# deepalcoholic/mlcomp

Measured on AMD Instinct MI355X. Metric: images/sec (whole node) ResNet-50 DAG train task, higher is better.
Workload: dtype bf16; 1 GPU; model=resnet50, global_batch=512, per_gpu_batch=512, image_size=224, parallelism=dp1, impl=native, optimizer=SGD momentum 0.9, wd 5e-5, fp32 master weights

## Files before the change

csrc/kernels/batchnorm.hip:

```cpp
#include "common.h"

namespace {

constexpr int NT = 256;

constexpr int FL = 8;
__global__ void __launch_bounds__(NT)
bn_finalize_kernel(const float* __restrict__ sum, const float* __restrict__ sumsq, int ncopy,
                   const float* __restrict__ gamma, const float* __restrict__ beta,
                   float* __restrict__ save_mean, float* __restrict__ save_invstd,
                   float* __restrict__ scale, float* __restrict__ shift,
                   float* __restrict__ run_mean, float* __restrict__ run_var,
                   long rows, int C, float eps, float momentum) {
  const int c = blockIdx.x * (NT / FL) + (threadIdx.x / FL), q = threadIdx.x % FL;
  float s1 = 0.f, s2 = 0.f;
  if (c < C) {
#pragma unroll 4
    for (int k = q; k < ncopy; k += FL) { s1 += sum[(long)k * C + c]; s2 += sumsq[(long)k * C + c]; }
  }
#pragma unroll
  for (int o = 1; o < FL; o <<= 1) { s1 += __shfl_xor(s1, o, 64); s2 += __shfl_xor(s2, o, 64); }
  if (c >= C || q != 0) return;
  const float inv_count = 1.f / (float)rows;
  const float mean = s1 * inv_count;
  const float var = fmaxf(s2 * inv_count - mean * mean, 0.f);
  const float inv = rsqrtf(var + eps);
  save_mean[c] = mean;
  save_invstd[c] = inv;
  const float g = gamma[c] * inv;
  scale[c] = g;
  shift[c] = beta[c] - mean * g;
  if (run_mean) {
    const float unbiased = rows > 1 ? var * (float)rows / (float)(rows - 1) : var;
    run_mean[c] = (1.f - momentum) * run_mean[c] + momentum * mean;
    run_var[c] = (1.f - momentum) * run_var[c] + momentum * unbiased;
  }
}

template <int U>
__global__ void __launch_bounds__(NT)
bn_fwd_apply_kernel(const bf16* __restrict__ y, const bf16* __restrict__ res, bf16* __restrict__ z,
                    const float* __restrict__ scale_, const float* __restrict__ shift_,
                    const float* __restrict__ rscale_, const float* __restrict__ rshift_,
                    long rows, int C, int relu) {
  const int G = C >> 3;
  const long gtid = (long)blockIdx.x * NT + threadIdx.x;
  const long stride = (long)gridDim.x * NT;
  const int cg = (int)(gtid % G);
  const int c0 = cg * 8;
  float scale[8], shift[8], rscale[8], rshift[8];
#pragma unroll
  for (int j = 0; j < 8; ++j) {
    scale[j] = scale_[c0 + j]; shift[j] = shift_[c0 + j];
    rscale[j] = rscale_ ? rscale_[c0 + j] : 1.f; rshift[j] = rscale_ ? rshift_[c0 + j] : 0.f;
  }
  const long total = rows * G;
  const long last = total - G + cg;
  for (long i0 = gtid; i0 < total; i0 += stride * U) {
    uint4 yv[U], rv[U];
#pragma unroll
    for (int u = 0; u < U; ++u) {
      const long i = min(i0 + u * stride, last);
      yv[u] = *reinterpret_cast<const uint4*>(y + i * 8);
      if (res) rv[u] = *reinterpret_cast<const uint4*>(res + i * 8);
    }
#pragma unroll
    for (int u = 0; u < U; ++u) {
      const long i = i0 + u * stride;
      float f[8];
      unpack8(yv[u], f);
#pragma unroll
      for (int j = 0; j < 8; ++j) f[j] = f[j] * scale[j] + shift[j];
      if (res) {
        float r[8];
        unpack8(rv[u], r);
#pragma unroll
        for (int j = 0; j < 8; ++j) f[j] += r[j] * rscale[j] + rshift[j];
      }
      if (relu) {
#pragma unroll
        for (int j = 0; j < 8; ++j) f[j] = fmaxf(f[j], 0.f);
      }
      if (i < total) *reinterpret_cast<uint4*>(z + i * 8) = pack8(f);
    }
  }
}

constexpr int NSTAT = 32;

__global__ void __launch_bounds__(NT)
bn_bwd_reduce_kernel(const bf16* __restrict__ dz, const bf16* __restrict__ z, const bf16* __restrict__ y,
                     const float* __restrict__ mean, float* __restrict__ sums, long rows, int C, int ncopy) {
  __shared__ float red[2][NT][9];
  const int G = C >> 3;
  const long gtid = (long)blockIdx.x * NT + threadIdx.x;
  const long stride = (long)gridDim.x * NT;
  const int cg = (int)(gtid % G);
  const int c0 = cg * 8;
  float mu[8], s1[8], s2[8];
#pragma unroll
  for (int j = 0; j < 8; ++j) { mu[j] = mean[c0 + j]; s1[j] = 0.f; s2[j] = 0.f; }
  const long total = rows * G;
  constexpr int U = 4;
  for (long i0 = gtid; i0 < total; i0 += stride * U) {
    uint4 dv[U], yv[U], zv[U];
#pragma unroll
    for (int u = 0; u < U; ++u) {
      const long i = i0 + u * stride;
      const long off = (i < total ? i : i0) * 8;
      dv[u] = ldg16(dz + off);
      yv[u] = ldg16(y + off);
      zv[u] = z ? ldg16(z + off) : make_uint4(0u, 0u, 0u, 0u);
    }
#pragma unroll
    for (int u = 0; u < U; ++u) {
      if (i0 + u * stride >= total) break;
      float d[8], yy[8];
      unpack8(dv[u], d);
      unpack8(yv[u], yy);
      if (z) {
        float zz[8];
        unpack8(zv[u], zz);
#pragma unroll
        for (int j = 0; j < 8; ++j) d[j] = zz[j] > 0.f ? d[j] : 0.f;
      }
#pragma unroll
      for (int j = 0; j < 8; ++j) { s1[j] += d[j]; s2[j] += d[j] * (yy[j] - mu[j]); }
    }
  }
  const int t = threadIdx.x;
#pragma unroll
  for (int j = 0; j < 8; ++j) { red[0][t][j] = s1[j]; red[1][t][j] = s2[j]; }
  __syncthreads();
  const int lanes = NT < G ? NT : G;
  const int base_cg = (int)(((long)blockIdx.x * NT) % G);
  float* dst = sums + (size_t)(blockIdx.x % ncopy) * 2 * C;
  if (t < lanes) {
    float a[8], b[8];
#pragma unroll
    for (int j = 0; j < 8; ++j) { a[j] = 0.f; b[j] = 0.f; }
    for (int u = t; u < NT; u += G) {
#pragma unroll
      for (int j = 0; j < 8; ++j) { a[j] += red[0][u][j]; b[j] += red[1][u][j]; }
    }
    const int cgt = (base_cg + t) % G;
#pragma unroll
    for (int j = 0; j < 8; ++j) {
      atomicAdd(dst + cgt * 8 + j, a[j]);
      atomicAdd(dst + C + cgt * 8 + j, b[j]);
    }
  }
}

__global__ void __launch_bounds__(NT)
bn_bwd_finalize_kernel(const float* __restrict__ sums, const float* __restrict__ invstd,
                       const float* __restrict__ gamma, float* __restrict__ coef,
                       float* __restrict__ dgamma, float* __restrict__ dbeta, long rows, int C, int ncopy) {
  const int c = blockIdx.x * (NT / FL) + (threadIdx.x / FL), q = threadIdx.x % FL;
  float S1 = 0.f, S2 = 0.f;
  if (c < C) {
#pragma unroll 4
    for (int k = q; k < ncopy; k += FL) {
      S1 += sums[(size_t)k * 2 * C + c];
      S2 += sums[(size_t)k * 2 * C + C + c];
    }
  }
#pragma unroll
  for (int o = 1; o < FL; o <<= 1) { S1 += __shfl_xor(S1, o, 64); S2 += __shfl_xor(S2, o, 64); }
  if (c >= C || q != 0) return;
  const float invM = 1.f / (float)rows;
  const float is = invstd[c];
  const float k1 = gamma[c] * is;
  coef[c] = k1;
  coef[C + c] = -k1 * S1 * invM;
  coef[2 * C + c] = -k1 * is * is * S2 * invM;
  if (dgamma) { dgamma[c] = S2 * is; dbeta[c] = S1; }
}

template <int U>
__global__ void __launch_bounds__(NT)
bn_bwd_apply_kernel(const bf16* __restrict__ dz, const bf16* __restrict__ z, const bf16* __restrict__ y,
                    const float* __restrict__ mean, const float* __restrict__ coef,
                    bf16* __restrict__ dy, bf16* __restrict__ dres, long rows, int C) {
  const int G = C >> 3;
  const long gtid = (long)blockIdx.x * NT + threadIdx.x;
  const long stride = (long)gridDim.x * NT;
  const int cg = (int)(gtid % G);
  const int c0 = cg * 8;
  float mu[8], k1[8], k2[8], k3[8];
#pragma unroll
  for (int j = 0; j < 8; ++j) {
    mu[j] = mean[c0 + j];
    k1[j] = coef[c0 + j];
    k2[j] = coef[C + c0 + j];
    k3[j] = coef[2 * C + c0 + j];
  }
  const long total = rows * G;
  const long last = total - G + cg;
  for (long i0 = gtid; i0 < total; i0 += stride * U) {
    uint4 dv[U], yv[U], zv[U];
#pragma unroll
    for (int u = 0; u < U; ++u) {
      const long i = min(i0 + u * stride, last);
      dv[u] = *reinterpret_cast<const uint4*>(dz + i * 8);
      yv[u] = *reinterpret_cast<const uint4*>(y + i * 8);
      if (z) zv[u] = *reinterpret_cast<const uint4*>(z + i * 8);
    }
#pragma unroll
    for (int u = 0; u < U; ++u) {
      const long i = i0 + u * stride;
      float d[8], yy[8], o[8];
      unpack8(dv[u], d);
      unpack8(yv[u], yy);
      if (z) {
        float zz[8];
        unpack8(zv[u], zz);
#pragma unroll
        for (int j = 0; j < 8; ++j) d[j] = zz[j] > 0.f ? d[j] : 0.f;
      }
      if (i < total) {
        if (dres) *reinterpret_cast<uint4*>(dres + i * 8) = pack8(d);
#pragma unroll
        for (int j = 0; j < 8; ++j) o[j] = k1[j] * d[j] + k2[j] + k3[j] * (yy[j] - mu[j]);
        *reinterpret_cast<uint4*>(dy + i * 8) = pack8(o);
      }
    }
  }
}

constexpr int FG = 32;

__device__ __forceinline__ void fused_geom(int G, int& gb, int& nslices) {
  gb = slice_groups(G, FG);
  nslices = G / gb;
}

__device__ __forceinline__ void fused_reduce(const float* __restrict__ a, const float* __restrict__ b, long stride,
                                             int ncopy, int c0, int nch, int t, float (&red)[2][NT]) {
  const int P = NT / nch, p = t / nch, cl = t % nch;
  float x = 0.f, y = 0.f;
  if (p < P) {
#pragma unroll 16
    for (int k = p; k < ncopy; k += P) { x += a[k * stride + c0 + cl]; y += b[k * stride + c0 + cl]; }
  }
  red[0][t] = x;
  red[1][t] = y;
  __syncthreads();
  if (t < nch) {
    for (int q = 1; q < P; ++q) { x += red[0][q * nch + t]; y += red[1][q * nch + t]; }
  }
  __syncthreads();
  if (t < nch) { red[0][t] = x; red[1][t] = y; }
  __syncthreads();
}

template <int U>
__global__ void __launch_bounds__(NT)
bn_fwd_fused_kernel(const bf16* __restrict__ y, const bf16* __restrict__ res, bf16* __restrict__ z,
                    const float* __restrict__ sum, const float* __restrict__ sumsq, int ncopy,
                    const float* __restrict__ gamma, const float* __restrict__ beta,
                    float* __restrict__ save_mean, float* __restrict__ save_invstd,
                    float* __restrict__ scale_out, float* __restrict__ shift_out,
                    float* __restrict__ run_mean, float* __restrict__ run_var,
                    const float* __restrict__ rscale_, const float* __restrict__ rshift_,
                    long rows, int C, float eps, float momentum, int relu) {
  __shared__ float lsc[FG * 8], lsh[FG * 8], red[2][NT];
  const int G = C >> 3;
  int gb, nslices;
  fused_geom(G, gb, nslices);
  const int slice = blockIdx.x % nslices, part = blockIdx.x / nslices, nparts = gridDim.x / nslices;
  const int t = threadIdx.x, nch = gb * 8, c0 = slice * nch;
  fused_reduce(sum, sumsq, (long)C, ncopy, c0, nch, t, red);
  if (t < nch) {
    const int c = c0 + t;
    const float s1 = red[0][t], s2 = red[1][t];
    const float inv_count = 1.f / (float)rows;
    const float mean = s1 * inv_count;
    const float var = fmaxf(s2 * inv_count - mean * mean, 0.f);
    const float inv = rsqrtf(var + eps);
    const float g = gamma[c] * inv, h = beta[c] - mean * g;
    lsc[t] = g;
    lsh[t] = h;
    if (part == 0) {
      save_mean[c] = mean;
      save_invstd[c] = inv;
      scale_out[c] = g;
      shift_out[c] = h;
      if (run_mean) {
        const float unbiased = rows > 1 ? var * (float)rows / (float)(rows - 1) : var;
        run_mean[c] = (1.f - momentum) * run_mean[c] + momentum * mean;
        run_var[c] = (1.f - momentum) * run_var[c] + momentum * unbiased;
      }
    }
  }
  __syncthreads();
  const int rpi = NT / gb;
  if (t >= rpi * gb) return;
  const int g = t % gb, cg = slice * gb + g;
  float sc[8], sh[8], rsc[8], rsh[8];
#pragma unroll
  for (int j = 0; j < 8; ++j) {
    sc[j] = lsc[g * 8 + j];
    sh[j] = lsh[g * 8 + j];
    rsc[j] = rscale_ ? rscale_[cg * 8 + j] : 1.f;
    rsh[j] = rscale_ ? rshift_[cg * 8 + j] : 0.f;
  }
  const long step = (long)nparts * rpi;
  for (long r0 = (long)part * rpi + t / gb; r0 < rows; r0 += step * U) {
    uint4 yv[U], rv[U];
#pragma unroll
    for (int u = 0; u < U; ++u) {
      const long r = min(r0 + u * step, rows - 1);
      yv[u] = ldg16(y + (r * G + cg) * 8);
      rv[u] = res ? ldg16(res + (r * G + cg) * 8) : make_uint4(0u, 0u, 0u, 0u);
    }
#pragma unroll
    for (int u = 0; u < U; ++u) {
      const long r = r0 + u * step;
      if (r >= rows) break;
      float f[8];
      unpack8(yv[u], f);
#pragma unroll
      for (int j = 0; j < 8; ++j) f[j] = f[j] * sc[j] + sh[j];
      if (res) {
        float q[8];
        unpack8(rv[u], q);
#pragma unroll
        for (int j = 0; j < 8; ++j) f[j] += q[j] * rsc[j] + rsh[j];
      }
      if (relu) {
#pragma unroll
        for (int j = 0; j < 8; ++j) f[j] = fmaxf(f[j], 0.f);
      }
      *reinterpret_cast<uint4*>(z + (r * G + cg) * 8) = pack8(f);
    }
  }
}

template <int U>
__global__ void __launch_bounds__(NT)
bn_bwd_fused_kernel(const bf16* __restrict__ dz, const bf16* __restrict__ z, const bf16* __restrict__ y,
                    const float* __restrict__ mean, const float* __restrict__ sums, int ncopy,
                    const float* __restrict__ invstd, const float* __restrict__ gamma,
                    float* __restrict__ dgamma, float* __restrict__ dbeta, bf16* __restrict__ dy,
                    bf16* __restrict__ dres, long rows, int C) {
  __shared__ float lk[3][FG * 8], lmu[FG * 8], red[2][NT];
  const int G = C >> 3;
  int gb, nslices;
  fused_geom(G, gb, nslices);
  const int slice = blockIdx.x % nslices, part = blockIdx.x / nslices, nparts = gridDim.x / nslices;
  const int t = threadIdx.x, nch = gb * 8, c0 = slice * nch;
  fused_reduce(sums, sums + C, 2L * C, ncopy, c0, nch, t, red);
  if (t < nch) {
    const int c = c0 + t;
    const float S1 = red[0][t], S2 = red[1][t];
    const float invM = 1.f / (float)rows;
    const float is = invstd[c];
    const float k1 = gamma[c] * is;
    lk[0][t] = k1;
    lk[1][t] = -k1 * S1 * invM;
    lk[2][t] = -k1 * is * is * S2 * invM;
    lmu[t] = mean[c];
    if (part == 0 && dgamma) { dgamma[c] = S2 * is; dbeta[c] = S1; }
  }
  __syncthreads();
  const int rpi = NT / gb;
  if (t >= rpi * gb) return;
  const int g = t % gb, cg = slice * gb + g;
  float k1[8], k2[8], k3[8], mu[8];
#pragma unroll
  for (int j = 0; j < 8; ++j) {
    k1[j] = lk[0][g * 8 + j];
    k2[j] = lk[1][g * 8 + j];
    k3[j] = lk[2][g * 8 + j];
    mu[j] = lmu[g * 8 + j];
  }
  const long step = (long)nparts * rpi;
  for (long r0 = (long)part * rpi + t / gb; r0 < rows; r0 += step * U) {
    uint4 dv[U], yv[U], zv[U];
#pragma unroll
    for (int u = 0; u < U; ++u) {
      const long r = min(r0 + u * step, rows - 1);
      const long i = r * G + cg;
      dv[u] = ldg16(dz + i * 8);
      yv[u] = ldg16(y + i * 8);
      zv[u] = z ? ldg16(z + i * 8) : make_uint4(0u, 0u, 0u, 0u);
    }
#pragma unroll
    for (int u = 0; u < U; ++u) {
      const long r = r0 + u * step;
      if (r >= rows) break;
      const long i = r * G + cg;
      float d[8], yy[8], o[8];
      unpack8(dv[u], d);
      unpack8(yv[u], yy);
      if (z) {
        float zz[8];
        unpack8(zv[u], zz);
#pragma unroll
        for (int j = 0; j < 8; ++j) d[j] = zz[j] > 0.f ? d[j] : 0.f;
      }
      if (dres) *reinterpret_cast<uint4*>(dres + i * 8) = pack8(d);
#pragma unroll
      for (int j = 0; j < 8; ++j) o[j] = k1[j] * d[j] + k2[j] + k3[j] * (yy[j] - mu[j]);
      *reinterpret_cast<uint4*>(dy + i * 8) = pack8(o);
    }
  }
}

int g_unroll = 1;
int g_max_blocks = 512;
int g_fused = 1;

long grid_mult(int G) {
  if (G > NT) return G / NT;
  int a = G, b = NT;
  while (b) { const int r = a % b; a = b; b = r; }
  return G / a;
}

int grid_for(long rows, int C) {
  const int G = C >> 3;
  long total = rows * G;
  long blocks = (total + NT * 4 - 1) / (NT * 4);
  if (blocks > g_max_blocks) blocks = g_max_blocks;
  if (blocks < 1) blocks = 1;
  const long m = grid_mult(G);
  blocks = ((blocks + m - 1) / m) * m;
  return (int)blocks;
}

int fused_grid(long rows, int C) {
  const int G = C >> 3;
  const int gb = slice_groups(G, FG), nslices = G / gb;
  const int rpi = NT / gb;
  long parts = (rows + (long)rpi * 4 - 1) / ((long)rpi * 4);
  long cap = g_max_blocks / nslices;
  if (cap < 1) cap = 1;
  if (parts > cap) parts = cap;
  if (parts < 1) parts = 1;
  return (int)(parts * nslices);
}

bool fused_ok(int C, int ncopy) {
  const int G = C >> 3;
  if (g_fused != 1 || C % 8 || ncopy < 1 || ncopy > 64) return false;
  return G >= 1;
}

bool shape_ok(int C) {
  const int G = C >> 3;
  if (C % 8) return false;
  return G <= NT || G % NT == 0;
}

}

int g_mlc_ncopy = NSTAT;
int g_mlc_det = 0;

MLC_EXPORT int mlc_set_deterministic(int det, int ncopy) {
  g_mlc_det = det ? 1 : 0;
  g_mlc_ncopy = ncopy >= NSTAT ? ncopy : NSTAT;
  return 0;
}
MLC_EXPORT int mlc_get_stat_copies() { return g_mlc_ncopy; }
MLC_EXPORT int mlc_get_deterministic() { return g_mlc_det; }

MLC_EXPORT int mlc_bn_finalize(const float* sum, const float* sumsq, int ncopy, const float* gamma,
                               const float* beta, float* save_mean, float* save_invstd, float* scale,
                               float* shift, float* run_mean, float* run_var, long rows, int C,
                               float eps, float momentum, hipStream_t st) {
  hipLaunchKernelGGL(bn_finalize_kernel, dim3((C + NT / FL - 1) / (NT / FL)), dim3(NT), 0, st, sum, sumsq, ncopy,
                     gamma, beta, save_mean, save_invstd, scale, shift, run_mean, run_var, rows, C, eps,
                     momentum);
  return hipGetLastError();
}

MLC_EXPORT int mlc_bn_fwd_apply2(const bf16* y, const bf16* res, bf16* z, const float* scale,
                                 const float* shift, const float* rscale, const float* rshift, long rows,
                                 int C, int relu, hipStream_t st) {
  if (!shape_ok(C) || (rscale && !rshift)) return -1;
  const dim3 grid(grid_for(rows, C));
  if (g_unroll >= 4)
    hipLaunchKernelGGL(bn_fwd_apply_kernel<4>, grid, dim3(NT), 0, st, y, res, z, scale, shift, rscale, rshift,
                       rows, C, relu);
  else if (g_unroll == 2)
    hipLaunchKernelGGL(bn_fwd_apply_kernel<2>, grid, dim3(NT), 0, st, y, res, z, scale, shift, rscale, rshift,
                       rows, C, relu);
  else
    hipLaunchKernelGGL(bn_fwd_apply_kernel<1>, grid, dim3(NT), 0, st, y, res, z, scale, shift, rscale, rshift,
                       rows, C, relu);
  return hipGetLastError();
}

MLC_EXPORT int mlc_bn_fwd_apply(const bf16* y, const bf16* res, bf16* z, const float* scale,
                                const float* shift, long rows, int C, int relu, hipStream_t st) {
  return mlc_bn_fwd_apply2(y, res, z, scale, shift, nullptr, nullptr, rows, C, relu, st);
}

MLC_EXPORT int mlc_bn_bwd_reduce(const bf16* dz, const bf16* z, const bf16* y, const float* mean,
                                 float* sums, long rows, int C, hipStream_t st) {
  if (!shape_ok(C)) return -1;
  int blocks = grid_for(rows, C);
  const int G = C >> 3;
  if (G >= 64) {
    int cap = 65536 / G;
    if (cap < 256) cap = 256;
    const long m = grid_mult(G);
    cap = (int)(((cap + m - 1) / m) * m);
    if (blocks > cap) blocks = cap;
  }
  if (g_mlc_det && blocks > g_mlc_ncopy) return -2;
  hipLaunchKernelGGL(bn_bwd_reduce_kernel, dim3(blocks), dim3(NT), 0, st, dz, z, y,
                     mean, sums, rows, C, g_mlc_ncopy);
  return hipGetLastError();
}

MLC_EXPORT int mlc_bn_bwd_finalize(const float* sums, const float* invstd, const float* gamma,
                                   float* coef, float* dgamma, float* dbeta, long rows, int C,
                                   hipStream_t st) {
  hipLaunchKernelGGL(bn_bwd_finalize_kernel, dim3((C + NT / FL - 1) / (NT / FL)), dim3(NT), 0, st, sums, invstd,
                     gamma, coef, dgamma, dbeta, rows, C, g_mlc_ncopy);
  return hipGetLastError();
}

MLC_EXPORT int mlc_bn_fwd_fused(const bf16* y, const bf16* res, bf16* z, const float* sum, const float* sumsq,
                                int ncopy, const float* gamma, const float* beta, float* save_mean,
                                float* save_invstd, float* scale, float* shift, float* run_mean, float* run_var,
                                const float* rscale, const float* rshift, long rows, int C, float eps,
                                float momentum, int relu, hipStream_t st) {
  if (!fused_ok(C, ncopy) || (rscale && !rshift) || rows < 1) return -1;
#define MLC_BNF(U) hipLaunchKernelGGL(bn_fwd_fused_kernel<U>, dim3(fused_grid(rows, C)), dim3(NT), 0, st, y, res, z, \
                                      sum, sumsq, ncopy, gamma, beta, save_mean, save_invstd, scale, shift, run_mean, \
                                      run_var, rscale, rshift, rows, C, eps, momentum, relu)
  if (g_unroll >= 4) MLC_BNF(4); else if (g_unroll == 2) MLC_BNF(2); else MLC_BNF(1);
#undef MLC_BNF
  return hipGetLastError();
}

MLC_EXPORT int mlc_bn_bwd_fused(const bf16* dz, const bf16* z, const bf16* y, const float* mean, const float* sums,
                                int ncopy, const float* invstd, const float* gamma, float* dgamma, float* dbeta,
                                bf16* dy, bf16* dres, long rows, int C, hipStream_t st) {
  if (!fused_ok(C, ncopy) || rows < 1) return -1;
#define MLC_BNB(U) hipLaunchKernelGGL(bn_bwd_fused_kernel<U>, dim3(fused_grid(rows, C)), dim3(NT), 0, st, dz, z, y, \
                                      mean, sums, ncopy, invstd, gamma, dgamma, dbeta, dy, dres, rows, C)
  if (g_unroll >= 4) MLC_BNB(4); else if (g_unroll == 2) MLC_BNB(2); else MLC_BNB(1);
#undef MLC_BNB
  return hipGetLastError();
}

MLC_EXPORT int mlc_bn_bwd_apply(const bf16* dz, const bf16* z, const bf16* y, const float* mean,
                                const float* coef, bf16* dy, bf16* dres, long rows, int C,
                                hipStream_t st) {
  if (!shape_ok(C)) return -1;
  const dim3 grid(grid_for(rows, C));
  if (g_unroll >= 4)
    hipLaunchKernelGGL(bn_bwd_apply_kernel<4>, grid, dim3(NT), 0, st, dz, z, y, mean, coef, dy, dres, rows, C);
  else if (g_unroll == 2)
    hipLaunchKernelGGL(bn_bwd_apply_kernel<2>, grid, dim3(NT), 0, st, dz, z, y, mean, coef, dy, dres, rows, C);
  else
    hipLaunchKernelGGL(bn_bwd_apply_kernel<1>, grid, dim3(NT), 0, st, dz, z, y, mean, coef, dy, dres, rows, C);
  return hipGetLastError();
}

MLC_EXPORT int mlc_bn_get_set(int key, int value) {
  int* k = key == 0 ? &g_unroll : key == 1 ? &g_max_blocks : key == 2 ? &g_fused : nullptr;
  if (!k) return -1;
  const int old = *k;
  if (value > 0) *k = value;
  return old;
}
```

csrc/kernels/common.h:

```cpp
#pragma once
#include <hip/hip_runtime.h>
#include <stdint.h>

typedef __bf16 bf16;
typedef __bf16 bf16x8 __attribute__((ext_vector_type(8)));
typedef __bf16 bf16x4 __attribute__((ext_vector_type(4)));
typedef __bf16 bf16x2 __attribute__((ext_vector_type(2)));
typedef short s16x4 __attribute__((ext_vector_type(4)));
typedef float f32x16 __attribute__((ext_vector_type(16)));
typedef float f32x4 __attribute__((ext_vector_type(4)));

#define LDS_PTR(T) __attribute__((address_space(3))) T*

#define MLC_EXPORT extern "C" __attribute__((visibility("default")))

extern int g_mlc_ncopy;
extern int g_mlc_det;
extern "C" int mlc_bn_stats(const bf16* x, float* sum, float* sumsq, long rows, int C, hipStream_t st);

static __device__ __forceinline__ float bf2f(bf16 v) { return (float)v; }
static __device__ __forceinline__ bf16 f2bf(float v) { return (bf16)v; }

static __host__ __device__ __forceinline__ int slice_groups(int G, int cap) {
  int d = G < cap ? G : cap;
  while (d > 1 && G % d) --d;
  return d;
}

static __device__ __forceinline__ void unpack8(const uint4& u, float* f) {
  const uint32_t w[4] = {u.x, u.y, u.z, u.w};
#pragma unroll
  for (int i = 0; i < 4; ++i) {
    f[2 * i] = __uint_as_float(w[i] << 16);
    f[2 * i + 1] = __uint_as_float(w[i] & 0xffff0000u);
  }
}

static __device__ __forceinline__ uint32_t pack2_bf16(float a, float b) {
  const bf16x2 r = {(bf16)a, (bf16)b};
  return __builtin_bit_cast(uint32_t, r);
}
static __device__ __forceinline__ uint32_t f2bf_bits(float f) {
  return (uint32_t)__builtin_bit_cast(unsigned short, (bf16)f);
}

static __device__ __forceinline__ uint4 pack8(const float* f) {
  uint4 r;
  r.x = pack2_bf16(f[0], f[1]);
  r.y = pack2_bf16(f[2], f[3]);
  r.z = pack2_bf16(f[4], f[5]);
  r.w = pack2_bf16(f[6], f[7]);
  return r;
}

static __device__ __forceinline__ uint4 ldg16(const void* p) {
  typedef unsigned u32x4 __attribute__((ext_vector_type(4)));
  const u32x4 v = *reinterpret_cast<const u32x4*>(p);
  return make_uint4(v.x, v.y, v.z, v.w);
}
static __device__ __forceinline__ void ldg8f(const float* p, float* f) {
  typedef float f32x4v __attribute__((ext_vector_type(4)));
  const f32x4v a = *reinterpret_cast<const f32x4v*>(p), b = *reinterpret_cast<const f32x4v*>(p + 4);
  f[0] = a.x; f[1] = a.y; f[2] = a.z; f[3] = a.w; f[4] = b.x; f[5] = b.y; f[6] = b.z; f[7] = b.w;
}

static __device__ __forceinline__ float wave_sum(float v) {
#pragma unroll
  for (int o = 32; o > 0; o >>= 1) v += __shfl_xor(v, o, 64);
  return v;
}

static __device__ __forceinline__ int xcd_remap(int orig, int nwg) {
  const int q = nwg >> 3, r = nwg & 7;
  const int xcd = orig & 7, loc = orig >> 3;
  return (xcd < r ? xcd * (q + 1) : r * (q + 1) + (xcd - r) * q) + loc;
}

static __global__ void __launch_bounds__(256) mlc_zero_f32_kernel(float* __restrict__ p, long n) {
  for (long i = (long)blockIdx.x * 256 + threadIdx.x; i < n; i += (long)gridDim.x * 256) p[i] = 0.f;
}
static inline void mlc_zero_f32(float* p, long n, hipStream_t st) {
  if (n <= 0) return;
  long blocks = (n + 255) / 256;
  if (blocks > 4096) blocks = 4096;
  hipLaunchKernelGGL(mlc_zero_f32_kernel, dim3(blocks), dim3(256), 0, st, p, n);
}
```

csrc/kernels/igemm.hip:

```cpp
#include "gfx950.h"
#include "convgeom.h"
#include <stdlib.h>
#include <map>
#include <mutex>
#include <vector>
#include <algorithm>
#include <cstdio>

namespace igemm {

constexpr int BK = 64, NTHR = 256;


template <int R>
__device__ __forceinline__ int mc_off(int k, int c) {
  if (R == 64) return k * 128 + ((c ^ (((k >> 1) & 1) << 2)) << 4);
  return k * (R * 2) + ((c ^ ((k & 3) << 2)) << 4);
}

template <class L, int R>
__device__ __forceinline__ void store_stage(char* lds, int tid, const uint4 (&v)[R / 32]) {
#pragma unroll
  for (int i = 0; i < R / 32; ++i) *reinterpret_cast<uint4*>(lds + L::lds_off(i, tid)) = v[i];
}
// ... 366 lines not shown
#pragma unroll
      for (int c = 0; c < NC; ++c) {
        const bool ok = (unsigned)(hb + st.rd[c]) < (unsigned)g.H && (unsigned)(wb + st.sd[c]) < (unsigned)g.W;
        v[2 * c + j] = bload(rsr, ok ? rel + st.coff[c] : OOB);
      }
    }
  }
};

struct BnIn { const float* sc; const float* sh; };
template <class L, class = void> struct HasXform { static constexpr bool value = false; };
template <class L> struct HasXform<L, decltype((void)L::XF)> { static constexpr bool value = L::XF; };
template <class L, class = void> struct HasDma { static constexpr bool value = false; };
template <class L> struct HasDma<L, decltype((void)L::DMA)> {
  static constexpr bool value = L::DMA && !HasXform<L>::value && !HasSum<L>::value;
};

__device__ __forceinline__ uint4 bn_relu8(uint4 v, const float* a, const float* b, bool ok) {
  float f[8];
  unpack8(v, f);
#pragma unroll
  for (int e = 0; e < 8; ++e) f[e] = fmaxf(f[e] * a[e] + b[e], 0.f);
  const uint4 r = pack8(f);
  return ok ? r : make_uint4(0u, 0u, 0u, 0u);
}

template <int R>
struct MatKCBn : MatKC<R> {
  static constexpr bool XF = true;
  BnIn bn;
  __device__ void xform(const typename MatKC<R>::St& st, int kt, int tid, uint4 (&v)[R / 32]) const {
    const int c0 = kt * BK + (tid & 7) * 8;
    const bool kv = c0 < this->K;
    float a[8], b[8];
    ldg8f(bn.sc + (kv ? c0 : 0), a);
    ldg8f(bn.sh + (kv ? c0 : 0), b);
#pragma unroll
    for (int i = 0; i < R / 32; ++i) v[i] = bn_relu8(v[i], a, b, kv && st.off[i] != OOB);
  }
};

template <int R>
struct ConvFwdABn : ConvFwdA<R> {
  static constexpr bool XF = true;
  BnIn bn;
  __device__ void xform(const typename ConvFwdA<R>::St& st, int kt, int tid, uint4 (&v)[R / 32]) const {
    const ConvGeom& g = this->g;
    const int k0 = kt * BK, k = k0 + (tid & 7) * 8;
    unsigned rs_, cc, rr, ss;
    if (g.C % BK == 0) {
      g.fC.divmod((unsigned)k0, rs_, cc);
      cc += (unsigned)(k - k0);
    } else {
      g.fC.divmod((unsigned)k, rs_, cc);
    }
    g.fKW.divmod(rs_, rr, ss);
    const bool kv = k < this->K;
    const unsigned P = kv ? tap_pat((int)rr, (int)ss) : NO_TAP;
    float a[8], b[8];
    ldg8f(bn.sc + (kv ? cc : 0), a);
    ldg8f(bn.sh + (kv ? cc : 0), b);
#pragma unroll
    for (int i = 0; i < R / 32; ++i) v[i] = bn_relu8(v[i], a, b, (st.msk[i] & P) == P);
  }
};

template <int R>
struct MatMCBn : MatMC<R> {
  static constexpr bool XF = true;
  BnIn bn;
  __device__ void xform(const typename MatMC<R>::St& st, int kt, int tid, uint4 (&v)[R / 32]) const {
    const int c0 = st.n0 + (tid % (R / 8)) * 8;
    const bool cv = c0 < this->cols;
    float a[8], b[8];
    ldg8f(bn.sc + (cv ? c0 : 0), a);
    ldg8f(bn.sh + (cv ? c0 : 0), b);
    const int left = this->K - kt * BK;
#pragma unroll
    for (int i = 0; i < R / 32; ++i) v[i] = bn_relu8(v[i], a, b, cv && MatMC<R>::kr(i, tid) < left);
  }
};

template <int R>
struct ConvWgradBBn : ConvWgradB<R> {
  static constexpr bool XF = true;
  BnIn bn;
  __device__ void xform(const typename ConvWgradB<R>::St& st, int kt, int tid, uint4 (&v)[R / 32]) const {
    constexpr int NC = ConvWgradB<R>::NC;
    const ConvGeom& g = this->g;
    const int p0 = kt * BK;
    unsigned t, w0, n0, h0;
    g.fWo.divmod((unsigned)p0, t, w0);
    g.fHo.divmod(t, n0, h0);
    int hb[2], wb[2];
#pragma unroll
    for (int j = 0; j < 2; ++j) {
      const int kr = (tid >> 3) + 32 * j;
      unsigned cw, wo, ch, ho;
      g.fWo.divmod(w0 + (unsigned)kr, cw, wo);
      g.fHo.divmod(h0 + cw, ch, ho);
      hb[j] = p0 + kr < this->P ? (int)ho * g.stride - g.pad : -(1 << 29);
      wb[j] = (int)wo * g.stride - g.padw;
    }
#pragma unroll
    for (int c = 0; c < NC; ++c) {
      float a[8], b[8];
      ldg8f(bn.sc + st.ci[c], a);
      ldg8f(bn.sh + st.ci[c], b);
#pragma unroll
      for (int j = 0; j < 2; ++j) {
        const bool ok = (unsigned)(hb[j] + st.rd[c]) < (unsigned)g.H && (unsigned)(wb[j] + st.sd[c]) < (unsigned)g.W;
        v[2 * c + j] = bn_relu8(v[2 * c + j], a, b, ok);
      }
    }
  }
};


struct IdentityRows {
  __device__ __forceinline__ size_t operator()(int m) const { return (size_t)m; }
};
struct ClassRows {
  DgradClass c; int H, W;
  __device__ __forceinline__ size_t operator()(int m) const {
    int n, i, j;
    c.decode(m, n, i, j);
    return ((size_t)n * H + i * c.S + c.ph) * W + j * c.S + c.pw;
  }
};
template <class Rows = IdentityRows>
struct StridedAddRows {
  Rows rows; int Ho, Wo; FastDiv fW, fH, fS;
  __device__ __forceinline__ size_t operator()(int m) const { return rows(m); }
  __device__ __forceinline__ bool addend_pixel(size_t pix, size_t& cpix) const {
    unsigned t, n, h, w, hq, hr, wq, wr;
    fW.divmod((unsigned)pix, t, w);
    fH.divmod(t, n, h);
    fS.divmod(h, hq, hr);
    fS.divmod(w, wq, wr);
    cpix = ((size_t)n * Ho + hq) * Wo + wq;
    return (hr | wr) == 0;
  }
};
template <class R> struct HasStridedAdd { static constexpr bool value = false; };
template <class R> struct HasStridedAdd<StridedAddRows<R>> { static constexpr bool value = true; };

struct BnBwdEpi {
  const bf16* mask = nullptr;
  const bf16* y0 = nullptr; const float* mean0 = nullptr; float* sums0 = nullptr;
  const bf16* y1 = nullptr; const float* mean1 = nullptr; float* sums1 = nullptr;
  const float* msc0 = nullptr; const float* msh0 = nullptr;
  const float* msc1 = nullptr; const float* msh1 = nullptr;
  int ncopy = NSTAT;
};

__device__ __forceinline__ float erf_from_exp(float x, float e) {
  const float t = __builtin_amdgcn_rcpf(1.f + 0.3275911f * fabsf(x));
  const float p = ((((1.061405429f * t - 1.453152027f) * t + 1.421413741f) * t - 0.284496736f) * t + 0.254829592f) * t;
  return copysignf(1.f - p * e, x);
}

__device__ __forceinline__ void dense_act8(float (&a)[8], int act, bf16* pre) {
  const int mode = act & 3;
  if (mode == 3) {
    if (pre) *reinterpret_cast<uint4*>(pre) = pack8(a);
#pragma unroll
    for (int e = 0; e < 8; ++e) a[e] = fmaxf(a[e], 0.f);
    return;
  }
  if (mode == 2) {
    float d[8];
#pragma unroll
    for (int e = 0; e < 8; ++e) {
      const float u = a[e];
      const float ex = __expf(-0.5f * u * u);
      const float cdf = 0.5f * (1.f + erf_from_exp(u * 0.70710678118654752f, ex));
      d[e] = cdf + u * 0.3989422804014327f * ex;
      a[e] = u * cdf;
    }
    if (pre) *reinterpret_cast<uint4*>(pre) = pack8(d);
    return;
  }
  if (pre) *reinterpret_cast<uint4*>(pre) = pack8(a);
  if (mode == 1) {
#pragma unroll
    for (int e = 0; e < 8; ++e)
      a[e] = 0.5f * a[e] * (1.f + erf_from_exp(a[e] * 0.70710678118654752f, __expf(-0.5f * a[e] * a[e])));
  }
}
__device__ __forceinline__ void dense_dact8(float (&a)[8], int act, uint4 zv) {
  float z[8];
  unpack8(zv, z);
  if (act & 4) {
#pragma unroll
    for (int e = 0; e < 8; ++e) a[e] *= z[e];
    return;
  }
  if ((act & 3) == 3) {
#pragma unroll
    for (int e = 0; e < 8; ++e) a[e] = z[e] > 0.f ? a[e] : 0.f;
    return;
  }
#pragma unroll
  for (int e = 0; e < 8; ++e) {
    const float ex = __expf(-0.5f * z[e] * z[e]);
    const float cdf = 0.5f * (1.f + erf_from_exp(z[e] * 0.70710678118654752f, ex));
    a[e] *= cdf + z[e] * 0.3989422804014327f * ex;
  }
}

template <class RowMap = IdentityRows, bool kDense = false>
struct EpiBF16 {
  bf16* out; int ld; float* sum; float* sumsq; RowMap rowmap; const bf16* addend = nullptr;
  BnBwdEpi bn = {};
  const float* bias = nullptr; int act = 0; bf16* preact = nullptr; const bf16* dact = nullptr;
  int ncopy = NSTAT;
  bool raw_sync = false;
  __device__ __forceinline__ void esync() const {
    if (raw_sync) lds_barrier();
    else __syncthreads();
  }
  template <int BM, int BN, int MI, int NI>
  __device__ void apply(f32x16 (&acc)[MI][NI], char* lds, int m0, int n0, int M, int N,
                        int wm, int wn, int lane, int tid) const {
    if (sum) {
      const int slot = (int)((unsigned)((m0 / 64) + wm) % (unsigned)ncopy);
#pragma unroll
      for (int j = 0; j < NI; ++j) {
        float s1 = 0.f, s2 = 0.f;
#pragma unroll
        for (int i = 0; i < MI; ++i)
#pragma unroll
          for (int r = 0; r < 16; ++r) { const float v = acc[i][j][r]; s1 += v; s2 += v * v; }
        s1 += __shfl_xor(s1, 32, 64);
        s2 += __shfl_xor(s2, 32, 64);
        const int n = n0 + wn * 32 * NI + 32 * j + lane;
        if (lane < 32 && n < N) {
          atomicAdd(sum + (size_t)slot * N + n, s1);
          atomicAdd(sumsq + (size_t)slot * N + n, s2);
        }
      }
    }
    constexpr int RS = (BN + 8) * 2;
    esync();
#pragma unroll
    for (int i = 0; i < MI; ++i)
#pragma unroll
      for (int j = 0; j < NI; ++j)
#pragma unroll
        for (int r = 0; r < 16; ++r) {
          const int m = wm * 32 * MI + 32 * i + (r & 3) + 8 * (r >> 2) + 4 * (lane >> 5);
          const int n = wn * 32 * NI + 32 * j + (lane & 31);
          *reinterpret_cast<bf16*>(lds + m * RS + n * 2) = (bf16)acc[i][j][r];
        }
    esync();
    constexpr int CPR = BN / 8;
    constexpr int RPI = NTHR / CPR;
    constexpr bool EXACT = RPI * CPR == NTHR && BM % RPI == 0;
    const bool tok = EXACT || tid < RPI * CPR;
    const int c = tid % CPR;
    const int nc = n0 + c * 8;
    const bool red = !kDense && bn.y0 != nullptr;
    float mu0[8], mu1[8], s1[8], s2[8], t2[8], ma0[8], mb0[8], ma1[8], mb1[8];
    const bool aff = red && !bn.mask && bn.msc0, aff1 = aff && bn.msc1;
    if (red) {
      const int ncl = nc < N ? nc : 0;
#pragma unroll
      for (int e = 0; e < 8; ++e) {
        s1[e] = 0.f; s2[e] = 0.f; t2[e] = 0.f;
        mu1[e] = 0.f; ma0[e] = 0.f; mb0[e] = 0.f; ma1[e] = 0.f; mb1[e] = 0.f;
      }
      ldg8f(bn.mean0 + ncl, mu0);
      if (bn.y1) ldg8f(bn.mean1 + ncl, mu1);
      if (aff) { ldg8f(bn.msc0 + ncl, ma0); ldg8f(bn.msh0 + ncl, mb0); }
      if (aff1) { ldg8f(bn.msc1 + ncl, ma1); ldg8f(bn.msh1 + ncl, mb1); }
    }
    const bool dense = kDense && (bias || act || dact);
    float bz[8];
#pragma unroll
    for (int e = 0; e < 8; ++e) bz[e] = 0.f;
    if (kDense && bias) ldg8f(bias + (nc < N ? nc : 0), bz);
    constexpr int ITERS = (BM + RPI - 1) / RPI;
    if (!addend && !red && !dense) {
#pragma unroll
      for (int it = 0; it < ITERS; ++it) {
        const int row = tid / CPR + RPI * it;
        const int m = m0 + row;
        if ((EXACT || (tok && row < BM)) && m < M && nc < N)
          *reinterpret_cast<uint4*>(out + rowmap(m) * ld + nc) =
              *reinterpret_cast<const uint4*>(lds + row * RS + c * 16);
      }
      return;
    }
    constexpr int UMAX = kDense ? 4 : 8;
    constexpr int U = ITERS < UMAX ? ITERS : UMAX;
    const bool has_add = addend != nullptr, has_mask = red && bn.mask, has_y1 = red && bn.y1;
    constexpr bool kSAdd = HasStridedAdd<RowMap>::value;
#pragma unroll 1
    for (int it0 = 0; it0 < ITERS; it0 += U) {
      constexpr int UB = kDense ? 1 : U;
      constexpr int UD = kDense ? U : 1;
      uint4 vv[U], aa[U], zz[UB], p0[UB], p1[UB], du[UD];
      size_t off[U];
      bool ok[U], hit[U];
#pragma unroll
      for (int u = 0; u < U; ++u) {
        int row = tid / CPR + RPI * (it0 + u);
        const bool rin = EXACT || (tok && row < BM);
        if (!rin) row = 0;
        const int m = m0 + row;
        ok[u] = rin && m < M && nc < N;
        const size_t pix = ok[u] ? rowmap(m) : 0;
        off[u] = ok[u] ? pix * ld + nc : 0;
        vv[u] = *reinterpret_cast<const uint4*>(lds + row * RS + c * 16);
        const uint4 zero = make_uint4(0u, 0u, 0u, 0u);
        if constexpr (kSAdd) {
          size_t cpix = 0;
          hit[u] = has_add && ok[u] && rowmap.addend_pixel(pix, cpix);
          aa[u] = hit[u] ? ldg16(addend + cpix * ld + nc) : zero;
        } else {
          hit[u] = has_add;
          aa[u] = has_add ? ldg16(addend + off[u]) : zero;
        }
        if constexpr (!kDense) {
          zz[u] = has_mask ? ldg16(bn.mask + off[u]) : zero;
          p0[u] = red ? ldg16(bn.y0 + off[u]) : zero;
          p1[u] = has_y1 ? ldg16(bn.y1 + off[u]) : zero;
        }
        if constexpr (kDense) du[u] = dact ? ldg16(dact + off[u]) : zero;
      }
#pragma unroll
      for (int u = 0; u < U; ++u) {
        if (!ok[u]) continue;
        uint4 v = vv[u];
        if (has_add || red || dense) {
          float a[8];
          unpack8(v, a);
          if constexpr (kDense) {
          if (bias) {
#pragma unroll
            for (int e = 0; e < 8; ++e) a[e] += bz[e];
          }
          dense_act8(a, act, preact ? preact + off[u] : nullptr);
          if (dact) dense_dact8(a, act, du[u]);
          }
          if (hit[u]) {
            float b[8];
            unpack8(aa[u], b);
#pragma unroll
            for (int e = 0; e < 8; ++e) a[e] += b[e];
          }
          if constexpr (!kDense) {
            if (has_mask) {
              float z[8];
              unpack8(zz[u], z);
#pragma unroll
              for (int e = 0; e < 8; ++e) a[e] = z[e] > 0.f ? a[e] : 0.f;
            } else if (aff) {
              float y[8], q[8];
              unpack8(p0[u], y);
#pragma unroll
              for (int e = 0; e < 8; ++e) q[e] = y[e] * ma0[e] + mb0[e];
              if (aff1) {
                unpack8(p1[u], y);
#pragma unroll
                for (int e = 0; e < 8; ++e) q[e] += y[e] * ma1[e] + mb1[e];
              }
#pragma unroll
              for (int e = 0; e < 8; ++e) a[e] = q[e] > 0.f ? a[e] : 0.f;
            }
          }
          v = pack8(a);
          if constexpr (!kDense) if (red) {
            unpack8(v, a);
            float y[8];
            unpack8(p0[u], y);
#pragma unroll
            for (int e = 0; e < 8; ++e) { s1[e] += a[e]; s2[e] += a[e] * (y[e] - mu0[e]); }
            if (has_y1) {
              unpack8(p1[u], y);
#pragma unroll
              for (int e = 0; e < 8; ++e) t2[e] += a[e] * (y[e] - mu1[e]);
            }
          }
        }
        *reinterpret_cast<uint4*>(out + off[u]) = v;
      }
    }
    if (red) {
      float* rb = reinterpret_cast<float*>(lds);
      esync();
#pragma unroll
      for (int e = 0; e < 8; ++e) {
        rb[tid * 24 + e] = s1[e];
        rb[tid * 24 + 8 + e] = s2[e];
        rb[tid * 24 + 16 + e] = t2[e];
      }
      esync();
      if (tid < BN) {
        const int col = tid, cc = col >> 3, e = col & 7, n = n0 + col;
        float a = 0.f, b = 0.f, d = 0.f;
        for (int r = 0; r < RPI; ++r) {
          const float* q = rb + (cc + CPR * r) * 24;
          a += q[e]; b += q[8 + e]; d += q[16 + e];
        }
        if (n < N) {
          const int slot = (int)((unsigned)(m0 / BM) % (unsigned)bn.ncopy);
          float* d0 = bn.sums0 + (size_t)slot * 2 * N;
          atomicAdd(d0 + n, a);
          atomicAdd(d0 + N + n, b);
          if (bn.y1) {
            float* d1 = bn.sums1 + (size_t)slot * 2 * N;
            atomicAdd(d1 + n, a);
            atomicAdd(d1 + N + n, d);
          }
        }
      }
    }
  }
};

struct EpiF32Slab {
  float* ws; int ld; size_t slab;
  template <int BM, int BN, int MI, int NI>
  __device__ void apply(f32x16 (&acc)[MI][NI], char*, int m0, int n0, int M, int N,
                        int wm, int wn, int lane, int) const {
    float* out = ws + (size_t)blockIdx.z * slab;
#pragma unroll
    for (int i = 0; i < MI; ++i)
#pragma unroll
      for (int j = 0; j < NI; ++j) {
        const int n = n0 + wn * 32 * NI + 32 * j + (lane & 31);
        if (n >= N) continue;
#pragma unroll
        for (int r = 0; r < 16; ++r) {
          const int m = m0 + wm * 32 * MI + 32 * i + (r & 3) + 8 * (r >> 2) + 4 * (lane >> 5);
          if (m < M) out[(size_t)m * ld + n] = acc[i][j][r];
        }
      }
  }
};


struct DenseFinish {
  bf16* C; int ldc; const float* bias; int act; bf16* preact; const bf16* addend; const bf16* dact;
  __device__ __forceinline__ void run(const float* ws, size_t slab, int splits, size_t src, int m, int c) const {
    typedef float v4 __attribute__((ext_vector_type(4)));
    const float* base = ws + src;
    v4 lo = {0.f, 0.f, 0.f, 0.f}, hi = {0.f, 0.f, 0.f, 0.f};
    int k = 0;
    for (; k + 2 <= splits; k += 2) {
      const v4 p0 = *reinterpret_cast<const v4*>(base + k * slab);
      const v4 q0 = *reinterpret_cast<const v4*>(base + k * slab + 4);
      const v4 p1 = *reinterpret_cast<const v4*>(base + (k + 1) * slab);
      const v4 q1 = *reinterpret_cast<const v4*>(base + (k + 1) * slab + 4);
      lo += p0 + p1;
      hi += q0 + q1;
    }
    if (k < splits) {
      lo += *reinterpret_cast<const v4*>(base + k * slab);
      hi += *reinterpret_cast<const v4*>(base + k * slab + 4);
    }
    float a[8] = {lo.x, lo.y, lo.z, lo.w, hi.x, hi.y, hi.z, hi.w};
    const size_t o = (size_t)m * ldc + c;
    if (bias) {
      float bz[8];
      ldg8f(bias + c, bz);
#pragma unroll
      for (int e = 0; e < 8; ++e) a[e] += bz[e];
    }
    dense_act8(a, act, preact ? preact + o : nullptr);
    if (dact) dense_dact8(a, act, ldg16(dact + o));
    if (addend) {
      float b[8];
      unpack8(ldg16(addend + o), b);
#pragma unroll
      for (int e = 0; e < 8; ++e) a[e] += b[e];
    }
    *reinterpret_cast<uint4*>(C + o) = pack8(a);
  }
};

struct EpiSlabFused {
  float* ws; int ld; size_t slab; unsigned* cnt;
  int dense;
  float* outf; int accumulate;
  DenseFinish fin;
  template <int BM, int BN, int MI, int NI>
  __device__ void apply(f32x16 (&acc)[MI][NI], char* lds, int m0, int n0, int M, int N,
                        int wm, int wn, int lane, int tid) const {
    float* part = ws + (size_t)blockIdx.z * slab;
#pragma unroll
    for (int i = 0; i < MI; ++i)
#pragma unroll
      for (int j = 0; j < NI; ++j) {
        const int n = n0 + wn * 32 * NI + 32 * j + (lane & 31);
        if (n >= N) continue;
#pragma unroll
        for (int r = 0; r < 16; ++r) {
          const int m = m0 + wm * 32 * MI + 32 * i + (r & 3) + 8 * (r >> 2) + 4 * (lane >> 5);
          if (m < M) part[(size_t)m * ld + n] = acc[i][j][r];
        }
      }
    vmwait<0>();
    __syncthreads();
    int* flag = reinterpret_cast<int*>(lds);
    if (tid == 0) {
      __builtin_amdgcn_fence(__ATOMIC_RELEASE, "agent");
      vmwait<0>();
      const unsigned t = __hip_atomic_fetch_add(cnt + blockIdx.x, 1u, __ATOMIC_RELAXED, __HIP_MEMORY_SCOPE_AGENT);
// ... 636 lines not shown

struct MkMatKC {
  const bf16* p; int ld, rows, K;
  template <int R> MatKC<R> make() const { return MatKC<R>{p, ld, rows, K}; }
};
struct MkMatMC {
  const bf16* p; int ld, K, cols;
  template <int R> MatMC<R> make() const { return MatMC<R>{p, ld, K, cols}; }
};
struct MkMatMCSum {
  const bf16* p; int ld, K, cols; float* colsum;
  template <int R> MatMCSum<R> make() const { return MatMCSum<R>{p, ld, K, cols, colsum}; }
};
struct MkMatKCBn {
  const bf16* p; int ld, rows, K; BnIn bn;
  template <int R> MatKCBn<R> make() const { return MatKCBn<R>{{p, ld, rows, K}, bn}; }
};
struct MkMatMCBn {
  const bf16* p; int ld, K, cols; BnIn bn;
  template <int R> MatMCBn<R> make() const { return MatMCBn<R>{{p, ld, K, cols}, bn}; }
};
struct MkConvFwdA {
  const bf16* x; ConvGeom g; int M, K;
  template <int R> ConvFwdA<R> make() const { return ConvFwdA<R>{x, g, M, K}; }
};
struct MkConvFwdABn {
  const bf16* x; ConvGeom g; int M, K; BnIn bn;
  template <int R> ConvFwdABn<R> make() const { return ConvFwdABn<R>{{x, g, M, K}, bn}; }
};
struct MkConvDgradA {
  const bf16* dy; ConvGeom g; int M, K; DgradClass cl;
  template <int R> ConvDgradA<R> make() const { return ConvDgradA<R>{dy, g, M, K, cl}; }
};
struct MkConvDgradB {
  const bf16* w; ConvGeom g; DgradClass cl;
  template <int R> ConvDgradB<R> make() const { return ConvDgradB<R>{w, g, cl}; }
};
struct MkConvDgradBT {
  const bf16* wt; ConvGeom g; DgradClass cl;
  template <int R> ConvDgradBT<R> make() const { return ConvDgradBT<R>{wt, g, cl}; }
};
struct MkConvWgradB {
  const bf16* x; ConvGeom g; int P, KK;
  template <int R> ConvWgradB<R> make() const { return ConvWgradB<R>{x, g, P, KK}; }
};
struct MkConvWgradBBn {
  const bf16* x; ConvGeom g; int P, KK; BnIn bn;
  template <int R> ConvWgradBBn<R> make() const { return ConvWgradBBn<R>{{x, g, P, KK}, bn}; }
};

template <class EPI, class FA, class FB>
static hipError_t launch_tiles(int tile, int M, int N, int K, int splits, hipStream_t st, const EPI& epi,
                               const FA& fa, const FB& fb) {
  if (tile == 1) return launch<256, 64>(fa.template make<256>(), fb.template make<64>(), epi, M, N, K, splits, st);
  if (tile == 2) return launch<64, 256>(fa.template make<64>(), fb.template make<256>(), epi, M, N, K, splits, st);
  if (tile == 3) return launch<256, 128>(fa.template make<256>(), fb.template make<128>(), epi, M, N, K, splits, st);
  if (tile == 4) return launch<128, 256>(fa.template make<128>(), fb.template make<256>(), epi, M, N, K, splits, st);
  return launch<128, 128>(fa.template make<128>(), fb.template make<128>(), epi, M, N, K, splits, st);
}

template <class EPI, class FA, class FB>
static hipError_t launch_dense_tiles(int dt, int M, int N, int K, int splits, hipStream_t st, const EPI& epi,
                                     const FA& fa, const FB& fb) {
  if (dt == 5) return launch<128, 96>(fa.template make<128>(), fb.template make<96>(), epi, M, N, K, splits, st);
  if (dt == 6) return launch<128, 192>(fa.template make<128>(), fb.template make<192>(), epi, M, N, K, splits, st);
  return launch<128, 288>(fa.template make<128>(), fb.template make<288>(), epi, M, N, K, splits, st);
}

template <class EPI>
static hipError_t dispatch_ab(int ta, int tb, const bf16* A, int lda, const bf16* B, int ldb, int tile, int M, int N,
                              int K, int splits, hipStream_t st, const EPI& epi) {
  const MkMatKC a_kc{A, lda, M, K}, b_kc{B, ldb, N, K};
  const MkMatMC a_mc{A, lda, K, M}, b_mc{B, ldb, K, N};
  if (!ta && tb) return launch_tiles(tile, M, N, K, splits, st, epi, a_kc, b_kc);
  if (!ta && !tb) return launch_tiles(tile, M, N, K, splits, st, epi, a_kc, b_mc);
  if (ta && tb) return launch_tiles(tile, M, N, K, splits, st, epi, a_mc, b_kc);
  return launch_tiles(tile, M, N, K, splits, st, epi, a_mc, b_mc);
}

MLC_EXPORT int mlc_bn_stat_copies() { return NSTAT; }

MLC_EXPORT int mlc_gemm_config(int prefetch) {
  const int old = igemm::g_prefetch;
  if (prefetch == 1 || prefetch == 2) igemm::g_prefetch = prefetch;
  return old;
}

MLC_EXPORT int mlc_gemm_get_set(int key, int value) {
  static int* const knobs[] = {
      &g_prefetch, &g_split_target, &g_split_target_mat, &g_big_tiles, &g_big_min_blocks, &g_single_stage,
      &g_splitk_fused, &g_dense_narrow, &g_gemm_dma, &g_split_target_dense, &g_dense_tile, &g_dense_split,
      &g_dense_bf16_split_target, &g_single_stage_kt, &g_persist, &g_persist_nbuf, &g_persist_kt};
  if (key < 0 || key >= (int)(sizeof(knobs) / sizeof(knobs[0]))) return -1;
  int* k = knobs[key];
  if (key == 14) resolve_persist_defaults();
  if (key == 10 || key == 11) {
    int sp = 1;
    (void)pick_dense_tile(4096, 768, 768, sp);
  }
  const int old = *k;
  if (key == 10) {
    if (value >= -1) *k = value;
    return old;
  }
  if (value >= 0 && (value > 0 || key == 3 || key == 5 || key == 6 || key == 7 || key == 8 || key == 12)) *k = value;
  return old;
}

static int conv_fwd_impl(const bf16* x, const bf16* w, bf16* y, int ldy, float* sum, float* sumsq,
                         int N, int H, int W, int C, int Co, int KH, int KW, int stride,
                         int pad, int dil, int Ho, int Wo, const float* in_sc, const float* in_sh,
                         hipStream_t st) {
  if (C % 8 || Co % 8 || ldy < Co || ldy % 8 || KH > 15 || KW > 16 || ((in_sc == nullptr) != (in_sh == nullptr)))
    return -1;
  const int M = N * Ho * Wo, K = KH * KW * C;
  const int tile = pick_tile(M, Co);
  EpiBF16<> epi{y, ldy, sum, sumsq, IdentityRows{}};
  epi.ncopy = g_mlc_ncopy;
  if (sum && g_mlc_det && (M + 63) / 64 > g_mlc_ncopy) return -2;
  const BnIn bn{in_sc, in_sh};
  const MkMatKC fb{w, K, Co, K};
  if (KH == 1 && KW == 1 && stride == 1 && pad == 0) {
    if (in_sc) return launch_tiles(tile, M, Co, K, 1, st, epi, MkMatKCBn{x, C, M, K, bn}, fb);
    return launch_tiles(tile, M, Co, K, 1, st, epi, MkMatKC{x, C, M, K}, fb);
  }
  const ConvGeom g = mkgeom(N, H, W, C, Co, KH, KW, stride, pad, dil, Ho, Wo);
  if (in_sc) return launch_tiles(tile, M, Co, K, 1, st, epi, MkConvFwdABn{x, g, M, K, bn}, fb);
  return launch_tiles(tile, M, Co, K, 1, st, epi, MkConvFwdA{x, g, M, K}, fb);
}

MLC_EXPORT int mlc_conv_fwd(const bf16* x, const bf16* w, bf16* y, float* sum, float* sumsq,
                            int N, int H, int W, int C, int Co, int KH, int KW, int stride,
                            int pad, int dil, int Ho, int Wo, const float* in_sc, const float* in_sh,
                            hipStream_t st) {
  return conv_fwd_impl(x, w, y, Co, sum, sumsq, N, H, W, C, Co, KH, KW, stride, pad, dil, Ho, Wo, in_sc, in_sh, st);
}

MLC_EXPORT int mlc_conv_fwd_ld(const bf16* x, const bf16* w, bf16* y, int ldy, int N, int H, int W, int C, int Co,
                               int KH, int KW, int stride, int pad, int dil, int Ho, int Wo, hipStream_t st) {
  return conv_fwd_impl(x, w, y, ldy, nullptr, nullptr, N, H, W, C, Co, KH, KW, stride, pad, dil, Ho, Wo, nullptr,
                       nullptr, st);
}

struct DgradAddend {
  const bf16* same = nullptr; const bf16* compact = nullptr; int S = 1;
};

static int dgrad_check(const BnBwdEpi& bn, const DgradAddend& add, int N, int H, int W, int C, int Co, int KH,
                       int KW, int stride, const float* sum, const float* sumsq) {
  if (C % 8 || Co % 8 || KH > 15 || KW > 16 || stride < 1 || ((sum == nullptr) != (sumsq == nullptr))) return -1;
  if (add.S < 1 || (add.compact && add.same)) return -1;
  if (bn.y0 && g_mlc_det && ((long)N * H * W + 63) / 64 > g_mlc_ncopy) return -2;
  if (bn.msc0 && (!bn.msh0 || !bn.y0 || (bn.msc1 && (!bn.msh1 || !bn.y1)))) return -1;
  if (bn.y0 && (!bn.mean0 || !bn.sums0 || (bn.y1 && (!bn.mean1 || !bn.sums1)))) return -1;
  return 0;
}

template <class Rows, class FA, class FB>
static hipError_t launch_dgrad(const Rows& rows, bf16* dx, const DgradAddend& add, const BnBwdEpi& bn, float* sum,
                               float* sumsq, int H, int W, int M, int C, int K, hipStream_t st, const FA& fa,
                               const FB& fb) {
  const int tile = pick_tile(M, C);
  if (add.compact) {
    const StridedAddRows<Rows> srows{rows, (H - 1) / add.S + 1, (W - 1) / add.S + 1, FastDiv(W), FastDiv(H),
                                     FastDiv(add.S)};
    EpiBF16<StridedAddRows<Rows>> epi{dx, C, sum, sumsq, srows, add.compact, bn};
    epi.ncopy = g_mlc_ncopy;
    return launch_tiles(tile, M, C, K, 1, st, epi, fa, fb);
  }
  EpiBF16<Rows> epi{dx, C, sum, sumsq, rows, add.same, bn};
  epi.ncopy = g_mlc_ncopy;
  return launch_tiles(tile, M, C, K, 1, st, epi, fa, fb);
}

template <class MkB>
static int dgrad_classes(const bf16* dy, const bf16* w, bf16* dx, const DgradAddend& add, const BnBwdEpi& bn,
                         const ConvGeom& g, int pad, float* sum, float* sumsq, hipStream_t st) {
  hipError_t err = hipSuccess;
  for (int ph = 0; ph < g.stride && ph < g.H; ++ph)
    for (int pw = 0; pw < g.stride && pw < g.W; ++pw) {
      const DgradClass cl = mkclass(g.stride, ph, pw, g.H, g.W, g.Ho, g.Wo, g.Co, g.KH, g.KW, pad, g.dil);
      if (cl.nr > 15 || cl.ns > 16) return -1;
      const int M = g.N * cl.Hc * cl.Wc, K = cl.nr * cl.ns * cl.ncb * BK;
      if (M <= 0) continue;
      if (sum && g_mlc_det && (M + 63) / 64 > g_mlc_ncopy) return -2;
      const MkConvDgradA fa{dy, g, M, K, cl};
      const MkB fb{w, g, cl};
      if (g.stride == 1)
        err = launch_dgrad(IdentityRows{}, dx, add, bn, sum, sumsq, g.H, g.W, M, g.C, K, st, fa, fb);
      else
        err = launch_dgrad(ClassRows{cl, g.H, g.W}, dx, add, bn, sum, sumsq, g.H, g.W, M, g.C, K, st, fa, fb);
      if (err != hipSuccess) return err;
    }
  return err;
}

static int conv_dgrad_impl(const bf16* dy, const bf16* w, bf16* dx, const DgradAddend& add, int N,
                           int H, int W, int C, int Co, int KH, int KW, int stride, int pad,
                           int dil, int Ho, int Wo, const bf16* bn_mask, const bf16* bn_y0,
                           const float* bn_mean0, float* bn_sums0, const bf16* bn_y1,
                           const float* bn_mean1, float* bn_sums1, const float* bn_msc0,
                           const float* bn_msh0, const float* bn_msc1, const float* bn_msh1,
                           float* sum, float* sumsq, hipStream_t st) {
  const BnBwdEpi bn{bn_mask, bn_y0, bn_mean0, bn_sums0, bn_y1, bn_mean1, bn_sums1,
                    bn_msc0, bn_msh0, bn_msc1, bn_msh1, g_mlc_ncopy};
  if (const int rc = dgrad_check(bn, add, N, H, W, C, Co, KH, KW, stride, sum, sumsq)) return rc;
  const ConvGeom g = mkgeom(N, H, W, C, Co, KH, KW, stride, pad, dil, Ho, Wo);
  if (KH == 1 && KW == 1 && stride == 1 && pad == 0) {
    const DgradClass cl = mkclass(1, 0, 0, H, W, Ho, Wo, Co, 1, 1, 0, dil);
    const int M = N * H * W, K = cl.ncb * BK;
    if (sum && g_mlc_det && (M + 63) / 64 > g_mlc_ncopy) return -2;
    return launch_dgrad(IdentityRows{}, dx, add, bn, sum, sumsq, H, W, M, C, K, st, MkMatKC{dy, Co, M, Co},
                        MkConvDgradB{w, g, cl});
  }
  return dgrad_classes<MkConvDgradB>(dy, w, dx, add, bn, g, pad, sum, sumsq, st);
}

MLC_EXPORT int mlc_conv_dgrad(const bf16* dy, const bf16* w, bf16* dx, const bf16* addend, int N,
                              int H, int W, int C, int Co, int KH, int KW, int stride, int pad,
                              int dil, int Ho, int Wo, const bf16* bn_mask, const bf16* bn_y0,
                              const float* bn_mean0, float* bn_sums0, const bf16* bn_y1,
                              const float* bn_mean1, float* bn_sums1, const float* bn_msc0,
                              const float* bn_msh0, const float* bn_msc1, const float* bn_msh1,
                              hipStream_t st) {
  return conv_dgrad_impl(dy, w, dx, DgradAddend{addend}, N, H, W, C, Co, KH, KW, stride, pad, dil, Ho, Wo, bn_mask,
                         bn_y0, bn_mean0, bn_sums0, bn_y1, bn_mean1, bn_sums1, bn_msc0, bn_msh0, bn_msc1, bn_msh1,
                         nullptr, nullptr, st);
}

MLC_EXPORT int mlc_conv_dgrad_sadd(const bf16* dy, const bf16* w, bf16* dx, const bf16* addend, const bf16* sadd,
                                   int sadd_stride, int N, int H, int W, int C, int Co, int KH, int KW,
                                   int stride, int pad, int dil, int Ho, int Wo, const bf16* bn_mask,
                                   const bf16* bn_y0, const float* bn_mean0, float* bn_sums0, const bf16* bn_y1,
                                   const float* bn_mean1, float* bn_sums1, const float* bn_msc0,
                                   const float* bn_msh0, const float* bn_msc1, const float* bn_msh1,
                                   hipStream_t st) {
  return conv_dgrad_impl(dy, w, dx, DgradAddend{addend, sadd, sadd_stride}, N, H, W, C, Co, KH, KW, stride, pad, dil,
                         Ho, Wo, bn_mask, bn_y0, bn_mean0, bn_sums0, bn_y1, bn_mean1, bn_sums1, bn_msc0, bn_msh0,
                         bn_msc1, bn_msh1, nullptr, nullptr, st);
}

MLC_EXPORT int mlc_conv_tr_fwd(const bf16* x, const bf16* w, bf16* y, float* sum, float* sumsq, int N, int Hi,
                               int Wi, int Cin, int Cout, int KH, int KW, int stride, int pad, int dil, int Ho,
                               int Wo, hipStream_t st) {
  int pad_h, pad_w;
  unpack_pad(pad, pad_h, pad_w);
  if (Hi != (Ho + 2 * pad_h - dil * (KH - 1) - 1) / stride + 1 || Wi != (Wo + 2 * pad_w - dil * (KW - 1) - 1) / stride + 1)
    return -1;
  return conv_dgrad_impl(x, w, y, DgradAddend{}, N, Ho, Wo, Cout, Cin, KH, KW, stride, pad, dil, Hi, Wi, nullptr,
                         nullptr, nullptr, nullptr, nullptr, nullptr, nullptr, nullptr, nullptr, nullptr,
                         nullptr, sum, sumsq, st);
}

static int conv_dgrad_t_impl(const bf16* dy, const bf16* wt, bf16* dx, const DgradAddend& add, int N,
                             int H, int W, int C, int Co, int KH, int KW, int stride, int pad,
                             int dil, int Ho, int Wo, const bf16* bn_mask, const bf16* bn_y0,
                             const float* bn_mean0, float* bn_sums0, const bf16* bn_y1,
                             const float* bn_mean1, float* bn_sums1, const float* bn_msc0,
                             const float* bn_msh0, const float* bn_msc1, const float* bn_msh1,
                             hipStream_t st) {
  const BnBwdEpi bn{bn_mask, bn_y0, bn_mean0, bn_sums0, bn_y1, bn_mean1, bn_sums1,
                    bn_msc0, bn_msh0, bn_msc1, bn_msh1, g_mlc_ncopy};
  if (const int rc = dgrad_check(bn, add, N, H, W, C, Co, KH, KW, stride, nullptr, nullptr)) return rc;
  int pad_h, pad_w;
  unpack_pad(pad, pad_h, pad_w);
  const int ph = dil * (KH - 1) - pad_h, pw = dil * (KW - 1) - pad_w;
  if (stride == 1 && ph >= 0 && pw >= 0) {
    if (Ho != H + 2 * pad_h - dil * (KH - 1) || Wo != W + 2 * pad_w - dil * (KW - 1)) return -1;
    const int M = N * H * W, K = KH * KW * Co;
    const MkMatKC fb{wt, K, C, K};
    if (KH == 1 && KW == 1)
      return launch_dgrad(IdentityRows{}, dx, add, bn, nullptr, nullptr, H, W, M, C, K, st, MkMatKC{dy, Co, M, Co},
                          fb);
    const ConvGeom gf = mkgeom(N, Ho, Wo, Co, C, KH, KW, 1, pack_pad(ph, pw), dil, H, W);
    return launch_dgrad(IdentityRows{}, dx, add, bn, nullptr, nullptr, H, W, M, C, K, st, MkConvFwdA{dy, gf, M, K},
                        fb);
  }
  const ConvGeom g = mkgeom(N, H, W, C, Co, KH, KW, stride, pad, dil, Ho, Wo);
  return dgrad_classes<MkConvDgradBT>(dy, wt, dx, add, bn, g, pad, nullptr, nullptr, st);
}

MLC_EXPORT int mlc_conv_dgrad_t(const bf16* dy, const bf16* wt, bf16* dx, const bf16* addend, int N,
                                int H, int W, int C, int Co, int KH, int KW, int stride, int pad,
                                int dil, int Ho, int Wo, const bf16* bn_mask, const bf16* bn_y0,
                                const float* bn_mean0, float* bn_sums0, const bf16* bn_y1,
                                const float* bn_mean1, float* bn_sums1, const float* bn_msc0,
                                const float* bn_msh0, const float* bn_msc1, const float* bn_msh1,
                                hipStream_t st) {
  return conv_dgrad_t_impl(dy, wt, dx, DgradAddend{addend}, N, H, W, C, Co, KH, KW, stride, pad, dil, Ho, Wo,
                           bn_mask, bn_y0, bn_mean0, bn_sums0, bn_y1, bn_mean1, bn_sums1, bn_msc0, bn_msh0, bn_msc1,
                           bn_msh1, st);
}

MLC_EXPORT int mlc_conv_dgrad_t_sadd(const bf16* dy, const bf16* wt, bf16* dx, const bf16* addend, const bf16* sadd,
                                     int sadd_stride, int N, int H, int W, int C, int Co, int KH, int KW,
                                     int stride, int pad, int dil, int Ho, int Wo, const bf16* bn_mask,
                                     const bf16* bn_y0, const float* bn_mean0, float* bn_sums0, const bf16* bn_y1,
                                     const float* bn_mean1, float* bn_sums1, const float* bn_msc0,
                                     const float* bn_msh0, const float* bn_msc1, const float* bn_msh1,
                                     hipStream_t st) {
  return conv_dgrad_t_impl(dy, wt, dx, DgradAddend{addend, sadd, sadd_stride}, N, H, W, C, Co, KH, KW, stride, pad,
                           dil, Ho, Wo, bn_mask, bn_y0, bn_mean0, bn_sums0, bn_y1, bn_mean1, bn_sums1, bn_msc0,
                           bn_msh0, bn_msc1, bn_msh1, st);
}

namespace {
__global__ void __launch_bounds__(256)
splitk_reduce_kernel(const float* __restrict__ ws, float* __restrict__ out, long n4, int splits,
                     long slab4, int accumulate) {
  typedef float v4 __attribute__((ext_vector_type(4)));
  const v4* w4 = reinterpret_cast<const v4*>(ws);
  v4* o4 = reinterpret_cast<v4*>(out);
  for (long i = (long)blockIdx.x * 256 + threadIdx.x; i < n4; i += (long)gridDim.x * 256) {
    v4 a = accumulate ? o4[i] : (v4){0.f, 0.f, 0.f, 0.f};
    v4 b = {0.f, 0.f, 0.f, 0.f};
    int k = 0;
    for (; k + 4 <= splits; k += 4) {
      const v4 u0 = w4[(k + 0) * slab4 + i], u1 = w4[(k + 1) * slab4 + i];
      const v4 u2 = w4[(k + 2) * slab4 + i], u3 = w4[(k + 3) * slab4 + i];
      a += u0 + u1;
      b += u2 + u3;
    }
    for (; k < splits; ++k) a += w4[k * slab4 + i];
    o4[i] = a + b;
  }
}
}

template <class FA, class FB>
static hipError_t launch_slabs_reduce(int tile, int M, int N, int K, int splits, hipStream_t st, float* ws,
                                      size_t slab, float* out, int accumulate, const FA& fa, const FB& fb) {
  const EpiF32Slab epi{ws, N, slab};
  const hipError_t e = launch_tiles(tile, M, N, K, splits, st, epi, fa, fb);
  if (e != hipSuccess) return e;
  const long n4 = (long)slab / 4;
  long blocks = (n4 + 255) / 256;
  if (blocks > 8192) blocks = 8192;
  hipLaunchKernelGGL(splitk_reduce_kernel, dim3(blocks), dim3(256), 0, st, ws, out, n4, splits, n4, accumulate);
  return hipGetLastError();
}

template <bool XF, class F>
static hipError_t with_wgrad_b(const bf16* x, const ConvGeom& g, int P, int KK, bool plain, const BnIn& bn, F f) {
  if constexpr (XF) {
    if (bn.sc) {
      if (plain) return f(MkMatMCBn{x, g.C, P, g.C, bn});
      return f(MkConvWgradBBn{x, g, P, KK, bn});
    }
  }
  if (plain) return f(MkMatMC{x, g.C, P, g.C});
  return f(MkConvWgradB{x, g, P, KK});
}

MLC_EXPORT int mlc_conv_wgrad_native(const bf16* dy, const bf16* x, float* dw, int N, int H, int W,
                              int C, int Co, int KH, int KW, int stride, int pad, int dil,
                              int Ho, int Wo, int splits, int accumulate, float* ws, long ws_floats,
                              const float* in_sc, const float* in_sh, hipStream_t st) {
  if (C % 8 || Co % 8 || ((in_sc == nullptr) != (in_sh == nullptr))) return -1;
  const BnIn bn{in_sc, in_sh};
  const int P = N * Ho * Wo, KK = KH * KW * C;
  const int tile = pick_tile(Co, KK);
  const bool plain = KH == 1 && KW == 1 && stride == 1 && pad == 0;
  const size_t slab = (size_t)Co * KK;
  bool use_slab = false;
  if (g_mlc_det) {
    splits = 1;
  } else if (splits <= 0) {
    const int ss = auto_splits(Co, KK, P, tile, g_split_target);
    use_slab = ws && slab >= (1u << 18) && (double)ss * slab * 4 >= 8e6 && (long)(ss * slab) <= ws_floats;
    splits = use_slab ? ss : auto_splits(Co, KK, P, tile, plain ? g_split_target_mat : g_split_target);
  } else {
    use_slab = ws && (long)(splits * slab) <= ws_floats;
  }
  const ConvGeom g = mkgeom(N, H, W, C, Co, KH, KW, stride, pad, dil, Ho, Wo);
  const MkMatMC fa{dy, Co, P, Co};
  if (use_slab) {
    splits = round_splits((P + BK - 1) / BK, splits);
    const int BMv = tile_bm(tile), BNv = tile_bn(tile);
    if (unsigned* cnt = split_counters(st, (long)((Co + BMv - 1) / BMv) * ((KK + BNv - 1) / BNv), splits, BMv, BNv)) {
      const EpiSlabFused epi{ws, KK, slab, cnt, 0, dw, accumulate, {}};
      return with_wgrad_b<true>(x, g, P, KK, plain, bn, [&](const auto& fb) {
        return launch_tiles(tile, Co, KK, P, splits, st, epi, fa, fb);
      });
    }
    return with_wgrad_b<true>(x, g, P, KK, plain, bn, [&](const auto& fb) {
      return launch_slabs_reduce(tile, Co, KK, P, splits, st, ws, slab, dw, accumulate, fa, fb);
    });
  }
  if (!accumulate) mlc_zero_f32(dw, (long)slab, st);
  const EpiF32Atomic epi{dw, KK};
  return with_wgrad_b<true>(x, g, P, KK, plain, bn, [&](const auto& fb) {
    return launch_tiles(tile, Co, KK, P, splits, st, epi, fa, fb);
  });
}

MLC_EXPORT int mlc_conv_fwd_ex(const bf16* x, const bf16* w, bf16* y, const float* bias, int act, int N, int H,
                               int W, int C, int Co, int KH, int KW, int stride, int pad, int dil, int Ho, int Wo,
                               hipStream_t st) {
  if (C % 8 || Co % 8 || KH > 15 || KW > 16) return -1;
  const int M = N * Ho * Wo, K = KH * KW * C;
  const int tile = pick_tile(M, Co);
  EpiBF16<IdentityRows, true> epi{y, Co, nullptr, nullptr, IdentityRows{}, nullptr};
  epi.bias = bias;
  epi.act = act;
  const MkMatKC fb{w, K, Co, K};
  if (KH == 1 && KW == 1 && stride == 1 && pad == 0)
    return launch_tiles(tile, M, Co, K, 1, st, epi, MkMatKC{x, C, M, K}, fb);
  const ConvGeom g = mkgeom(N, H, W, C, Co, KH, KW, stride, pad, dil, Ho, Wo);
  return launch_tiles(tile, M, Co, K, 1, st, epi, MkConvFwdA{x, g, M, K}, fb);
}

MLC_EXPORT int mlc_conv_fwd_res(const bf16* x, const bf16* w, bf16* y, const float* bias, int act,
                                const bf16* addend, int lda, int N, int H, int W, int C, int Co, int KH, int KW,
                                int stride, int pad, int dil, int Ho, int Wo, hipStream_t st) {
  if (C % 8 || Co % 8 || KH > 15 || KW > 16 || (act != 0 && act != 3)) return -1;
  if (addend && (lda < Co || lda % 8)) return -1;
  const int M = N * Ho * Wo, K = KH * KW * C;
  const int tile = pick_tile(M, Co);
  const EpiRes epi{y, Co, bias, addend, lda, act == 3};
  const MkMatKC fb{w, K, Co, K};
  if (KH == 1 && KW == 1 && stride == 1 && pad == 0)
    return launch_tiles(tile, M, Co, K, 1, st, epi, MkMatKC{x, C, M, K}, fb);
  const ConvGeom g = mkgeom(N, H, W, C, Co, KH, KW, stride, pad, dil, Ho, Wo);
  return launch_tiles(tile, M, Co, K, 1, st, epi, MkConvFwdA{x, g, M, K}, fb);
}

MLC_EXPORT int mlc_conv_wgrad_bias(const bf16* dy, const bf16* x, float* dw, float* dbias, int N, int H, int W,
                                   int C, int Co, int KH, int KW, int stride, int pad, int dil, int Ho, int Wo,
                                   int accumulate, float* ws, long ws_floats, hipStream_t st) {
  if (C % 8 || Co % 8 || !dbias) return -1;
  const int P = N * Ho * Wo, KK = KH * KW * C;
  const int tile = pick_tile(Co, KK);
  const bool plain = KH == 1 && KW == 1 && stride == 1 && pad == 0;
  const size_t slab = (size_t)Co * KK;
  int splits = g_mlc_det ? 1 : auto_splits(Co, KK, P, tile, plain ? g_split_target_mat : g_split_target);
  const ConvGeom g = mkgeom(N, H, W, C, Co, KH, KW, stride, pad, dil, Ho, Wo);
  const MkMatMCSum fa{dy, Co, P, Co, dbias};
  if (ws && splits > 1 && (long)(splits * slab) <= ws_floats) {
    splits = round_splits((P + BK - 1) / BK, splits);
    return with_wgrad_b<false>(x, g, P, KK, plain, BnIn{}, [&](const auto& fb) {
      return launch_slabs_reduce(tile, Co, KK, P, splits, st, ws, slab, dw, accumulate, fa, fb);
    });
  }
  if (!accumulate) mlc_zero_f32(dw, (long)slab, st);
  const EpiF32Atomic epi{dw, KK};
  return with_wgrad_b<false>(x, g, P, KK, plain, BnIn{}, [&](const auto& fb) {
    return launch_tiles(tile, Co, KK, P, splits, st, epi, fa, fb);
  });
}

MLC_EXPORT int mlc_gemm_f32out(const bf16* A, const bf16* B, float* C, const float* bias,
                               int M, int N, int K, int lda, int ldb, int ldc, int ta, int tb,
                               int out_mode, int accumulate, int splits, hipStream_t st) {
  if (K % 8 || lda % 8 || ldb % 8 || (ta && M % 8) || (!tb && N % 8)) return -1;
  const int tile = pick_tile(M, N);
  if (out_mode == 1) {
// ... 107 lines not shown
```

mlcomp_amd/ops/_lib.py:

```python
from __future__ import annotations

import ctypes as C
import os
import threading

import torch

_LIB = None
_LOCK = threading.Lock()

DETERMINISTIC = os.environ.get('MLC_DETERMINISTIC', '0') == '1'
DET_COPIES = max(32, int(os.environ.get('MLC_DET_COPIES', '4096')))

vp, i32, i64, f32, u32 = C.c_void_p, C.c_int, C.c_long, C.c_float, C.c_uint

_SIGS = {
    'mlc_conv_fwd': [vp, vp, vp, vp, vp] + [i32] * 12 + [vp, vp, vp],
    'mlc_conv_fwd_ld': [vp, vp, vp] + [i32] * 13 + [vp],
    'mlc_conv_dgrad': [vp] * 4 + [i32] * 12 + [vp] * 11 + [vp],
    'mlc_conv_dgrad_t': [vp] * 4 + [i32] * 12 + [vp] * 11 + [vp],
    'mlc_conv_dgrad_sadd': [vp] * 5 + [i32] * 13 + [vp] * 11 + [vp],
    'mlc_conv_dgrad_t_sadd': [vp] * 5 + [i32] * 13 + [vp] * 11 + [vp],
    'mlc_bilinear_up_fwd': [vp, vp] + [i32] * 6 + [vp],
    'mlc_bilinear_up_bwd': [vp, vp] + [i32] * 6 + [vp],
    'mlc_gn_relu_fwd': [vp, vp, vp, vp, vp] + [i32] * 4 + [f32, vp],
    'mlc_gn_relu_bwd': [vp] * 7 + [i32] * 4 + [f32, vp],
    'mlc_conv_tr_fwd': [vp] * 5 + [i32] * 12 + [vp],
    'mlc_wt_transpose': [vp, i32, i64, vp],
    'mlc_conv_wgrad': [vp, vp, vp] + [i32] * 14 + [vp, i64, vp, vp, vp],
    'mlc_conv_wgrad_native': [vp, vp, vp] + [i32] * 14 + [vp, i64, vp, vp, vp],
    'mlc_gemm_f32out': [vp, vp, vp, vp] + [i32] * 11 + [vp],
    'mlc_gemm_bf16out': [vp, vp, vp] + [i32] * 8 + [vp],
    'mlc_gemm256_nt': [vp, vp, vp, vp] + [i32] * 6 + [vp, i32, vp, vp, i32, i32, vp],
    'mlc_g256_dense': [vp, vp, vp] + [i32] * 7 + [vp, i32, vp, vp, vp, i32, vp],
    'mlc_gemm256_tn': [vp, vp, vp] + [i32] * 8 + [vp],
    'mlc_conv256_fwd': [vp] * 5 + [i32] * 13 + [vp],
    'mlc_augment': [vp, vp, vp, vp] + [i32] * 7 + [vp],
    'mlc_augment_seg': [vp] * 6 + [i32] * 9 + [vp],
    'mlc_augment_clip': [vp, vp, vp, vp] + [i32] * 8 + [vp],
    'mlc_gemm_bf16_ex': [vp, vp, vp] + [i32] * 8 + [vp, i32, vp, vp, vp, vp, i64, vp],
    'mlc_gemm_bf16_ex_native': [vp, vp, vp] + [i32] * 8 + [vp, i32, vp, vp, vp, vp, i64, vp],
    'mlc_ln_fwd': [vp] * 8 + [i32, i32, f32, f32, f32, vp, u32, u32, vp],
    'mlc_ln_bwd': [vp] * 10 + [i32, i32, f32, f32, vp, u32, u32, vp],
    'mlc_ln_finalize_many': [vp, i32, i32, vp],
    'mlc_embed_bwd': [vp] * 7 + [i32] * 4 + [vp],
    'mlc_softmax_fwd': [vp] * 4 + [i64, i32, i32, f32, f32, vp, u32, vp],
    'mlc_softmax_bwd': [vp] * 3 + [i64, i32, f32, f32, vp, u32, vp],
    'mlc_linear_wgrad_bias': [vp] * 4 + [i32] * 7 + [vp, i64, vp],
    'mlc_linear_wgrad_bias_native': [vp] * 4 + [i32] * 7 + [vp, i64, vp],
    'mlc_blaslt_mode': [i32],
    'mlc_blaslt_choices': [vp, i32],
    'mlc_upcat_fwd': [vp, vp, vp] + [i32] * 5 + [vp],
    'mlc_upcat_bwd': [vp, vp, vp] + [i32] * 5 + [vp],
    'mlc_seg_head_fwd': [vp] * 6 + [i64, i32, i32, vp],
    'mlc_seg_head_bwd': [vp] * 8 + [i64, i32, i32, f32, f32, f32, vp],
    'mlc_attn_fwd': [vp] * 4 + [i32, i32, i32, f32, f32, vp, u32, vp],
    'mlc_attn_bwd': [vp] * 5 + [i32, i32, i32, f32, f32, vp, u32, vp],
    'mlc_flash_fwd': [vp] * 4 + [i32] * 4 + [f32, f32, vp, u32, vp],
    'mlc_flash_bwd': [vp] * 7 + [i32] * 4 + [f32, f32, vp, u32, vp],
    'mlc_flash_fwd_masked': [vp] * 4 + [i32] * 4 + [f32, f32, vp, u32, i32, vp, i64, i64, vp],
    'mlc_flash_bwd_masked': [vp] * 7 + [i32] * 4 + [f32, f32, vp, u32, i32, vp, i64, i64, vp],
    'mlc_flash_bwd128': [i32],
    'mlc_colsum_acc': [vp, vp, vp, i32, i32, vp],
    'mlc_dropout': [vp, vp, i64, f32, vp, u32, vp],
    'mlc_bn_stat_copies': [],
    'mlc_set_deterministic': [i32, i32],
    'mlc_get_stat_copies': [],
    'mlc_get_deterministic': [],
    'mlc_gemm_config': [i32],
    'mlc_gemm_get_set': [i32, i32],
    'mlc_bn_get_set': [i32, i32],
    'mlc_bn_finalize': [vp, vp, i32] + [vp] * 8 + [i64, i32, f32, f32, vp],
    'mlc_bn_fwd_apply': [vp] * 5 + [i64, i32, i32, vp],
    'mlc_bn_fwd_apply2': [vp] * 7 + [i64, i32, i32, vp],
    'mlc_bn_bwd_reduce': [vp] * 5 + [i64, i32, vp],
    'mlc_bn_bwd_finalize': [vp] * 6 + [i64, i32, vp],
    'mlc_bn_fwd_fused': [vp] * 5 + [i32] + [vp] * 10 + [i64, i32, f32, f32, i32, vp],
    'mlc_bn_bwd_fused': [vp] * 5 + [i32] + [vp] * 6 + [i64, i32, vp],
    'mlc_bnact_fused': [vp] * 5 + [i32] + [vp] * 10 + [i64, i32, f32, f32, i32, f32, vp, i64, vp, i32, vp, i64, vp],
    'mlc_bn_bwd_apply': [vp] * 7 + [i64, i32, vp],
    'mlc_conv1x1_bn_bwd': [vp] * 18 + [i64, i32, i32, vp],
    'mlc_conv1x1_bn_bwd_ok': [i32, i32],
    'mlc_conv1x1_bwd_get_set': [i32, i32],
    'mlc_conv1x1_fwd': [vp] * 5 + [i64, i32, i32, vp],
    'mlc_conv1x1_fwd_ok': [i32, i32],
    'mlc_conv1x1_fwd_get_set': [i32, i32],
    'mlc_conv1x1_fwd_res': [vp] * 4 + [i32, vp, i32, i64, i32, i32, vp],
    'mlc_conv1x1_fwd_res_ok': [i32, i32],
    'mlc_maxpool_fwd': [vp, vp, vp] + [i32] * 9 + [vp],
    'mlc_maxpool_bwd': [vp, vp, vp] + [i32] * 9 + [vp],
    'mlc_stem_pool_fwd': [vp] * 6 + [i32] * 4 + [vp],
    'mlc_stem_pool_bwd_reduce_pooled': [vp] * 5 + [i32] * 4 + [vp],
    'mlc_stem_pool_bwd_reduce': [vp] * 5 + [i32] * 4 + [vp],
    'mlc_stem_pool_bwd_apply': [vp] * 6 + [i32] * 4 + [vp],
    'mlc_stem_s2d': [vp, vp] + [i32] * 5 + [vp],
    'mlc_stem_conv_fwd': [vp] * 5 + [i32] * 3 + [vp],
    'mlc_avgpool_fwd': [vp, vp, i32, i32, i32, vp],
    'mlc_avgpool_bwd': [vp, vp, vp, i32, i32, i32, vp],
    'mlc_avgpool2d_fwd': [vp, vp] + [i32] * 10 + [vp],
    'mlc_avgpool2d_bwd': [vp, vp, vp] + [i32] * 10 + [vp],
    'mlc_adaptive_avg_fwd': [vp, vp] + [i32] * 6 + [vp],
    'mlc_adaptive_avg_bwd': [vp, vp] + [i32] * 6 + [vp],
    'mlc_softmax_ce': [vp] * 5 + [i32, i32, i32, f32, f32, vp],
    'mlc_colsum': [vp, vp, i32, i32, vp],
    'mlc_nchw_to_nhwc': [vp, vp, i32, i32, i32, i32, vp],
    'mlc_cast_f32_bf16': [vp, vp, i64, vp],
    'mlc_sgd': [vp] * 5 + [i64, i64, i64, f32, f32, f32, i32, i32, vp],
    'mlc_adam': [vp] * 6 + [i64, i64, i64, f32, f32, f32, f32, i32, vp],
    'mlc_sqnorm': [vp, i64, vp, f32, vp],
    'mlc_opt_config': [i32, i32],
    'mlc_gconv_wb_elems': [i32] * 6,
    'mlc_gconv_fwd': [vp] * 6 + [i32] * 13 + [vp],
    'mlc_gconv_dgrad': [vp] * 4 + [i32] * 13 + [vp],
    'mlc_gconv_wgrad': [vp] * 3 + [i32] * 14 + [vp],
    'mlc_dwconv_fwd': [vp] * 5 + [i32] * 11 + [vp],
    'mlc_dwconv_dgrad': [vp] * 3 + [i32] * 11 + [vp],
    'mlc_dwconv_wgrad': [vp] * 4 + [i32] * 12 + [vp],
    'mlc_bn_stats': [vp, vp, vp, i64, i32, vp],
    'mlc_zero4': [vp, i64, vp, i64, vp, i64, vp, i64, vp],
    'mlc_bn_stats_ld': [vp, vp, vp, i64, i32, i32, i64, vp],
    'mlc_bnact_apply': [vp] * 7 + [i64, i32, i32, f32, vp, i64, vp],
    'mlc_bnact_bwd_reduce': [vp] * 10 + [i64, i32, i32, f32, vp, i64, i64, vp],
    'mlc_bnact_bwd': [vp] * 12 + [i64] + [vp] * 5 + [i64, i32, i32, f32, vp, i64, vp, i64, i64, vp, i32, vp],
    'mlc_bnact_bwd_apply': [vp] * 12 + [i64, i32, i32, f32, vp, i64, vp, i64, i64, vp, i32, vp],
    'mlc_act_fwd': [vp, vp, i64, i32, f32, vp],
    'mlc_act_bwd': [vp] * 4 + [i64, i32, f32, vp],
    'mlc_chscale_fwd': [vp] * 4 + [i32, i64, i32, i32, vp],
    'mlc_chscale_bwd': [vp] * 8 + [i32] * 3 + [vp],
    'mlc_conv_fwd_ex': [vp] * 4 + [i32] * 13 + [vp],
    'mlc_conv_fwd_res': [vp] * 4 + [i32, vp] + [i32] * 13 + [vp],
    'mlc_conv_wgrad_bias': [vp] * 4 + [i32] * 13 + [vp, i64, vp],
    'mlc_temporal_unfold': [vp, vp] + [i32] * 9 + [vp],
    'mlc_temporal_fold': [vp, vp, vp] + [i32] * 9 + [vp],
    'mlc_counters_owner': [i32],
    'mlc_counters_release': [i32],
    'mlc_counters_in_use': [],
    'mlc_comm_unique_id_bytes': [],
    'mlc_comm_get_unique_id': [vp],
    'mlc_comm_init': [vp, i32, i32, i32, i32, vp],
    'mlc_comm_async_error': [vp],
    'mlc_comm_abort': [vp],
    'mlc_comm_error_string': [i32],
    'mlc_comm_last_error': [vp],
    'mlc_comm_set_timeout': [i64],
    'mlc_comm_destroy': [vp],
    'mlc_allreduce': [vp, vp, vp, i64, i32, i32, vp],
    'mlc_broadcast': [vp, vp, vp, i64, i32, i32, vp],
    'mlc_reduce_scatter': [vp, vp, vp, i64, i32, i32, vp],
    'mlc_allgather': [vp, vp, vp, i64, i32, vp],
    'mlc_alltoall': [vp, vp, vp, i64, i32, i32, i32, vp],
}
_RESTYPE = {'mlc_comm_init': vp, 'mlc_gconv_wb_elems': C.c_long, 'mlc_counters_owner': None,
            'mlc_counters_release': C.c_long, 'mlc_counters_in_use': C.c_long,
            'mlc_comm_error_string': C.c_char_p, 'mlc_comm_last_error': C.c_char_p, 'mlc_comm_set_timeout': None}


def lib_path():
    from mlcomp_amd.build import KERNEL_LIB
    return os.environ.get('MLC_KERNEL_LIB') or KERNEL_LIB


def load():
    global _LIB
    if _LIB is not None:
        return _LIB
    with _LOCK:
        if _LIB is not None:
            return _LIB
        path = lib_path()
        if not os.path.exists(path):
            from mlcomp_amd.build import build_kernels
            build_kernels()
        lib = C.CDLL(path)
        for name, args in _SIGS.items():
            fn = getattr(lib, name)
            fn.argtypes = args
            fn.restype = _RESTYPE.get(name, C.c_int)
        for key, env in ((1, 'MLC_SPLIT_TARGET'), (2, 'MLC_SPLIT_TARGET_MAT'), (3, 'MLC_GEMM_BIG'),
                         (4, 'MLC_GEMM_BIG_MIN'), (5, 'MLC_GEMM_SINGLE_STAGE'), (6, 'MLC_SPLITK_FUSED'),
                         (9, 'MLC_SPLIT_TARGET_DENSE'), (12, 'MLC_DENSE_SPLIT_TARGET'), (13, 'MLC_SINGLE_STAGE_KT'),
                         (15, 'MLC_GEMM_PERSIST_NBUF'), (16, 'MLC_GEMM_PERSIST_KT')):
            if os.environ.get(env):
                lib.mlc_gemm_get_set(key, int(os.environ[env]))
        for key, env in ((0, 'MLC_BN_UNROLL'), (1, 'MLC_BN_BLOCKS')):
            if os.environ.get(env):
                lib.mlc_bn_get_set(key, int(os.environ[env]))
        if os.environ.get('MLC_FUSE_1X1_BLOCKS'):
            lib.mlc_conv1x1_bwd_get_set(0, int(os.environ['MLC_FUSE_1X1_BLOCKS']))
        if os.environ.get('MLC_CONV1X1_FWD_BLOCKS'):
            lib.mlc_conv1x1_fwd_get_set(0, int(os.environ['MLC_CONV1X1_FWD_BLOCKS']))
        if DETERMINISTIC:
            lib.mlc_set_deterministic(1, DET_COPIES)
            torch.use_deterministic_algorithms(True, warn_only=True)
        _LIB = lib
    return _LIB


def available() -> bool:
    return torch.cuda.is_available()


def stream():
    return C.c_void_p(torch.cuda.current_stream().cuda_stream)


def ptr(t):
    if t is None:
        return None
    return C.c_void_p(t.data_ptr())


def call(name, *args):
    rc = getattr(load(), name)(*args)
    if rc == -2 and DETERMINISTIC:
        raise RuntimeError(f'{name}: deterministic mode needs more partial-sum copies than '
                           f'MLC_DET_COPIES={DET_COPIES} (one per contributing block; raise it)')
    if rc != 0:
        raise RuntimeError(f'{name} failed (rc={rc}); check shape constraints '
                           f'(channels % 8 == 0) or HIP error')
    return rc
```

mlcomp_amd/ops/functional.py:

```python
from __future__ import annotations

from typing import Optional, Tuple

import contextlib
import math
import os
import threading

import torch
import torch.nn.functional as F

from . import _lib


def _cuda(t):
    return t is not None and t.is_cuda


def conv_out_hw(H, W, KH, KW, stride, pad, dil):
    ph, pw = (pad, pad) if isinstance(pad, int) else tuple(pad)
    Ho = (H + 2 * ph - dil * (KH - 1) - 1) // stride + 1
    Wo = (W + 2 * pw - dil * (KW - 1) - 1) // stride + 1
    return Ho, Wo


def pack_pad(pad) -> int:
    if isinstance(pad, int):
        return pad
    ph, pw = (int(v) for v in pad)
    return ph if ph == pw else (1 << 30) | (pw << 15) | ph


def bn_relu_input(x: torch.Tensor, in_affine) -> torch.Tensor:
    sc, sh = in_affine
    return torch.relu(x.float() * sc + sh).to(torch.bfloat16)


def conv2d_fwd(x: torch.Tensor, w: torch.Tensor, stride=1, pad=0, dil=1,
               stats: Optional[Tuple[torch.Tensor, torch.Tensor]] = None,
               out: Optional[torch.Tensor] = None, in_affine=None) -> torch.Tensor:
    N, H, W, C = x.shape
    Co, KH, KW, Ci = w.shape
    assert Ci == C, (w.shape, x.shape)
    Ho, Wo = conv_out_hw(H, W, KH, KW, stride, pad, dil)
    if _cuda(x):
        y = out if out is not None else torch.empty(N, Ho, Wo, Co, device=x.device, dtype=torch.bfloat16)
        ldy = rows_ld(y)
        if ldy != Co:
            assert ldy is not None and stats is None and in_affine is None, (y.shape, y.stride())
            _lib.call('mlc_conv_fwd_ld', _lib.ptr(x), _lib.ptr(w), _lib.ptr(y), ldy, N, H, W, C, Co, KH, KW, stride,
                      pack_pad(pad), dil, Ho, Wo, _lib.stream())
            return y
        s1, s2 = (stats if stats is not None else (None, None))
        sc, sh = in_affine if in_affine is not None else (None, None)
        _lib.call('mlc_conv_fwd', _lib.ptr(x), _lib.ptr(w), _lib.ptr(y), _lib.ptr(s1), _lib.ptr(s2),
                  N, H, W, C, Co, KH, KW, stride, pack_pad(pad), dil, Ho, Wo, _lib.ptr(sc), _lib.ptr(sh), _lib.stream())
        return y
    if in_affine is not None:
        x = bn_relu_input(x, in_affine)
    yf = F.conv2d(x.permute(0, 3, 1, 2).float(), w.permute(0, 3, 1, 2).float(), None, stride, pad, dil)
    if stats is not None:
        stats[0][:Co].add_(yf.sum(dim=(0, 2, 3)))
        stats[1][:Co].add_((yf * yf).sum(dim=(0, 2, 3)))
    y = yf.permute(0, 2, 3, 1).to(torch.bfloat16).contiguous()
    if out is not None:
        out.copy_(y)
        return out
    return y


CONV1X1_FWD = os.environ.get('MLC_CONV1X1_FWD', '1') == '1'


def conv1x1_fwd_available(Cin, Cout) -> bool:
    return not _lib.DETERMINISTIC and bool(_lib.load().mlc_conv1x1_fwd_ok(Cin, Cout))


def conv1x1_fwd(x: torch.Tensor, w: torch.Tensor, stats: Tuple[torch.Tensor, torch.Tensor],
                out: Optional[torch.Tensor] = None) -> torch.Tensor:
    Co, KH, KW, Ci = w.shape
    assert (KH, KW) == (1, 1) and x.shape[-1] == Ci and stats is not None, (w.shape, x.shape)
    if not _cuda(x):
        return conv2d_fwd(x, w, stats=stats, out=out)
    y = out if out is not None else torch.empty(*x.shape[:-1], Co, device=x.device, dtype=torch.bfloat16)
    assert y.is_contiguous() and x.is_contiguous(), (y.stride(), x.stride())
    _lib.call('mlc_conv1x1_fwd', _lib.ptr(x), _lib.ptr(w), _lib.ptr(y), _lib.ptr(stats[0]), _lib.ptr(stats[1]),
              x.numel() // Ci, Ci, Co, _lib.stream())
    return y


CONV1X1_RES = os.environ.get('MLC_CONV1X1_RES', '1') == '1'
CONV1X1_RES_MIN_ROWS_DEFAULT = {(128, 512): 25088, (256, 1024): 6272}
CONV1X1_RES_MIN_ROWS = (int(os.environ['MLC_CONV1X1_RES_MIN_ROWS'])
                        if os.environ.get('MLC_CONV1X1_RES_MIN_ROWS') else None)


def conv1x1_res_min_rows(Cin, Cout):
    if CONV1X1_RES_MIN_ROWS is not None:
        return CONV1X1_RES_MIN_ROWS
    return CONV1X1_RES_MIN_ROWS_DEFAULT.get((Cin, Cout))


def conv1x1_fwd_res_available(Cin, Cout) -> bool:
    return bool(_lib.load().mlc_conv1x1_fwd_res_ok(Cin, Cout))


def conv1x1_fwd_res(x: torch.Tensor, w: torch.Tensor, bias: Optional[torch.Tensor] = None,
                    addend: Optional[torch.Tensor] = None, act: int = 0,
                    out: Optional[torch.Tensor] = None) -> torch.Tensor:
    Co, KH, KW, Ci = w.shape
    assert (KH, KW) == (1, 1) and x.shape[-1] == Ci, (w.shape, x.shape)
    assert act in (0, 3), act
    if addend is not None:
        assert tuple(addend.shape) == (*x.shape[:-1], Co) and addend.dtype == torch.bfloat16, \
            (addend.shape, addend.dtype)
    if not _cuda(x):
        z = conv2d_fwd_res(x, w, bias, addend, act)
        if out is not None:
            out.copy_(z)
            return out
        return z
    assert x.dtype == torch.bfloat16 and x.is_contiguous(), (x.dtype, x.stride())
    assert w.dtype == torch.bfloat16 and w.is_contiguous() and w.device == x.device, (w.dtype, w.stride(), w.device)
    assert bias is None or (bias.dtype == torch.float32 and bias.is_contiguous() and bias.device == x.device
                            and bias.numel() == Co), (bias.dtype, bias.shape, bias.device)
    assert addend is None or addend.device == x.device, addend.device
    lda = 0
    if addend is not None:
        lda = rows_ld(addend)
        assert lda is not None and lda % 8 == 0 and addend.data_ptr() % 16 == 0, (addend.shape, addend.stride())
    y = out if out is not None else torch.empty(*x.shape[:-1], Co, device=x.device, dtype=torch.bfloat16)
    assert y.dtype == torch.bfloat16 and y.is_contiguous() and y.device == x.device \
        and tuple(y.shape) == (*x.shape[:-1], Co), (y.dtype, y.shape, y.stride(), y.device)
    _lib.call('mlc_conv1x1_fwd_res', _lib.ptr(x), _lib.ptr(w), _lib.ptr(y), _lib.ptr(bias), int(act),
              _lib.ptr(addend), lda, x.numel() // Ci, Ci, Co, _lib.stream())
    return y


def conv_transpose2d_fwd(x: torch.Tensor, w: torch.Tensor, out_hw, stride=2, pad=1, dil=1,
                         stats: Optional[Tuple[torch.Tensor, torch.Tensor]] = None) -> torch.Tensor:
    N, Hi, Wi, Cin = x.shape
    Cw, KH, KW, Cout = w.shape
    assert Cw == Cin, (w.shape, x.shape)
    Ho, Wo = out_hw
    assert conv_out_hw(Ho, Wo, KH, KW, stride, pad, dil) == (Hi, Wi), (out_hw, x.shape)
    if _cuda(x):
        y = torch.empty(N, Ho, Wo, Cout, device=x.device, dtype=torch.bfloat16)
        s1, s2 = (stats if stats is not None else (None, None))
        _lib.call('mlc_conv_tr_fwd', _lib.ptr(x), _lib.ptr(w), _lib.ptr(y), _lib.ptr(s1), _lib.ptr(s2),
                  N, Hi, Wi, Cin, Cout, KH, KW, stride, pack_pad(pad), dil, Ho, Wo, _lib.stream())
        return y
    oph = Ho - ((Hi - 1) * stride - 2 * pad + dil * (KH - 1) + 1)
    opw = Wo - ((Wi - 1) * stride - 2 * pad + dil * (KW - 1) + 1)
    yf = F.conv_transpose2d(x.permute(0, 3, 1, 2).float(), w.permute(0, 3, 1, 2).float(), None, stride, pad,
                            (oph, opw), 1, dil)
    if stats is not None:
        stats[0][:Cout].add_(yf.sum(dim=(0, 2, 3)))
        stats[1][:Cout].add_((yf * yf).sum(dim=(0, 2, 3)))
    return yf.permute(0, 2, 3, 1).to(torch.bfloat16).contiguous()


class BnBwdSpec:

    def __init__(self, mask, ys, affine=None):
        assert 1 <= len(ys) <= 2
        assert affine is None or (mask is None and len(affine) == len(ys))
        self.mask = mask
        self.ys = list(ys)
        self.affine = list(affine) if affine is not None else None


def wt_flip_transpose(w: torch.Tensor) -> torch.Tensor:
    return w.flip(1, 2).permute(3, 1, 2, 0).contiguous()


def dgrad_as_fwd_conv(KH, KW, stride, pad, dil) -> bool:
    return stride == 1 and pad <= dil * (KH - 1) and dil * (KH - 1) - pad == dil * (KW - 1) - pad


class WtTable:

    def __init__(self):
        self.slots = []
        self.views = []
        self.buf = None
        self.desc = None
        self.blocks = 0
        self._srcs = None

    def add(self, slot) -> int:
        self.slots.append(slot)
        return len(self.slots) - 1

    def __getitem__(self, i) -> torch.Tensor:
        return self.views[i]

    @staticmethod
    def _dims(shape):
        return tuple(shape) if len(shape) == 4 else (shape[0], 1, 1, shape[1])

    def finalize(self, device):
        if not self.slots:
            return
        total = sum((s.numel + 63) // 64 * 64 for s in self.slots)
        self.buf = torch.zeros(total, device=device, dtype=torch.bfloat16)
        off = 0
        for s in self.slots:
            Co, KH, KW, Ci = self._dims(s.shape)
            v = self.buf[off:off + s.numel]
            self.views.append(v.view(Ci, KH, KW, Co) if len(s.shape) == 4 else v.view(Ci, Co))
            off += (s.numel + 63) // 64 * 64
        if self.buf.is_cuda:
            self._build()

    def _build(self):
        rows, blk = [], 0
        for s, v in zip(self.slots, self.views):
            Co, KH, KW, Ci = self._dims(s.shape)
            rows.append([s.bf16.data_ptr(), v.data_ptr(), Co, KH * KW, Ci, blk])
            blk += KH * KW * ((Co + 63) // 64) * ((Ci + 63) // 64)
        self.desc = torch.tensor(rows, dtype=torch.int64).to(self.buf.device)
        self.blocks = blk
        self._srcs = [r[0] for r in rows]

    def refresh(self):
        if self.buf is None:
            return
        if not self.buf.is_cuda:
            for s, v in zip(self.slots, self.views):
                v.copy_(wt_flip_transpose(s.bf16) if s.bf16.dim() == 4 else s.bf16.t())
            return
        if self._srcs != [s.bf16.data_ptr() for s in self.slots]:
            self._build()
        _lib.call('mlc_wt_transpose', _lib.ptr(self.desc), len(self.slots), self.blocks, _lib.stream())


def conv2d_dgrad(dy: torch.Tensor, w: torch.Tensor, x_shape, stride=1, pad=0, dil=1,
                 addend: Optional[torch.Tensor] = None, out: Optional[torch.Tensor] = None,
                 bn: Optional[BnBwdSpec] = None, wt: Optional[torch.Tensor] = None,
                 strided_addend: Optional[Tuple[torch.Tensor, int]] = None) -> torch.Tensor:
    N, H, W, C = x_shape
    Co, KH, KW, Ci = w.shape
    _, Ho, Wo, _ = dy.shape
    if strided_addend is not None:
        assert addend is None, 'one addend form at a time'
        sadd, S = strided_addend
        assert S >= 1 and tuple(sadd.shape) == (N, (H - 1) // S + 1, (W - 1) // S + 1, C), (sadd.shape, x_shape, S)
        assert sadd.is_contiguous() and (out is None or out.data_ptr() != sadd.data_ptr())
    if _cuda(dy):
        dx = out if out is not None else torch.empty(N, H, W, C, device=dy.device, dtype=torch.bfloat16)
        b = [None] * 11
        if bn is not None:
            b[0] = bn.mask
            for k, (yk, mk, sk) in enumerate(bn.ys):
                b[1 + 3 * k:4 + 3 * k] = [yk, mk, sk]
            for k, (ak, hk) in enumerate(bn.affine or []):
                b[7 + 2 * k:9 + 2 * k] = [ak, hk]
        name, filt = 'mlc_conv_dgrad', w
        if wt is not None:
            assert tuple(wt.shape) == (Ci, KH, KW, Co), (wt.shape, w.shape)
            name, filt = 'mlc_conv_dgrad_t', wt
        add = [_lib.ptr(addend)]
        if strided_addend is not None:
            name, add = name + '_sadd', [None, _lib.ptr(sadd), S]
        _lib.call(name, _lib.ptr(dy), _lib.ptr(filt), _lib.ptr(dx), *add, N, H, W, C, Co, KH, KW, stride,
                  pack_pad(pad), dil, Ho, Wo, *[_lib.ptr(t) for t in b], _lib.stream())
        return dx
    if wt is not None and isinstance(pad, int) and dgrad_as_fwd_conv(KH, KW, stride, pad, dil):
        dxf = F.conv2d(dy.permute(0, 3, 1, 2).float(), wt.permute(0, 3, 1, 2).float(), None, 1,
                       dil * (KH - 1) - pad, dil)
    else:
        if wt is not None:
            w = wt_flip_transpose(wt)
        dxf = torch.nn.grad.conv2d_input((N, C, H, W), w.permute(0, 3, 1, 2).float(),
                                         dy.permute(0, 3, 1, 2).float(), stride, pad, dil)
    dxf = dxf.permute(0, 2, 3, 1)
    if addend is not None:
        dxf = dxf + addend.float()
    if strided_addend is not None:
        dxf = dxf.contiguous()
        dxf[:, ::S, ::S, :] += sadd.float()
    if bn is not None:
        if bn.mask is not None:
            dxf = dxf * (bn.mask.float() > 0)
        elif bn.affine is not None:
            q = sum(yk.float() * ak + hk for (yk, _, _), (ak, hk) in zip(bn.ys, bn.affine))
            dxf = dxf * (q > 0)
        d = dxf.to(torch.bfloat16).float().reshape(-1, C)
        for yk, mk, sk in bn.ys:
            sv = sk.view(NSTAT, 2, C)
            sv[0, 0] += d.sum(0)
            sv[0, 1] += (d * (yk.float().reshape(-1, C) - mk)).sum(0)
    dx = dxf.to(torch.bfloat16).contiguous()
    if out is not None:
        out.copy_(dx)
        return out
    return dx


_USE_SLAB = os.environ.get('MLC_WGRAD_SLAB', '1') != '0'
_SLAB = {}
_SLAB_OLD = []


_ROLE = threading.local()


def register_side_stream(stream) -> None:
    """Kept for callers of the old API: the workspace role is now explicit (side_role)."""


@contextlib.contextmanager
def side_stream(stream):
    prev = getattr(_ROLE, 'side', False)
    _ROLE.side = True
    try:
        with torch.cuda.stream(stream):
            yield
    finally:
        _ROLE.side = prev


class CounterLease:
    _next = 0

    def __init__(self, device):
        CounterLease._next += 1
        self.owner = CounterLease._next
        self.device = torch.device(device)

    def release(self):
        if self.owner and torch.cuda.is_available():
            from . import _lib
            with torch.cuda.device(self.device):
                _lib.load().mlc_counters_release(self.owner)
        self.owner = 0

    def __del__(self):
        try:
            self.release()
        except Exception:
            pass


@contextlib.contextmanager
def capture_scope(store: dict):
    prev = getattr(_ROLE, 'capture', None)
    _ROLE.capture = store
    lease = None
    if torch.cuda.is_available():
        from . import _lib
        lease = store.setdefault('__counter_lease__', CounterLease(torch.cuda.current_device()))
        _lib.load().mlc_counters_owner(lease.owner)
    try:
        yield
    finally:
        _ROLE.capture = prev
        if lease is not None:
            _lib.load().mlc_counters_owner(0)


def workspace_key(device) -> str:
    device = torch.device(device)
    if device.type == 'cuda' and getattr(_ROLE, 'side', False):
        return f'{device}/side'
    return str(device)


def workspace_store(pool: dict) -> dict:
    cap = getattr(_ROLE, 'capture', None)
    if cap is not None and torch.cuda.is_available() and torch.cuda.is_current_stream_capturing():
        return cap.setdefault(id(pool), {})
    return pool


def slab_workspace(device, n: int) -> torch.Tensor:
    key = workspace_key(device)
    store = workspace_store(_SLAB)
    buf = store.get(key)
    if buf is None or buf.numel() < n:
        if buf is not None:
            _SLAB_OLD.append(buf)
        buf = torch.empty(max(n, 1 << 20), device=device, dtype=torch.float32)
        store[key] = buf
    return buf


def conv2d_wgrad(dy: torch.Tensor, x: torch.Tensor, w_shape, stride=1, pad=0, dil=1,
                 out: Optional[torch.Tensor] = None, accumulate=False, in_affine=None,
                 slab: Optional[bool] = None) -> torch.Tensor:
    Co, KH, KW, Ci = w_shape
    N, H, W, C = x.shape
    _, Ho, Wo, _ = dy.shape
    if _cuda(dy):
        dw = out if out is not None else torch.empty(Co, KH, KW, Ci, device=dy.device, dtype=torch.float32)
        use = _USE_SLAB if slab is None else slab
        ws = slab_workspace(dy.device, min(32 * Co * KH * KW * Ci, 64 << 20)) if use else None
        sc, sh = in_affine if in_affine is not None else (None, None)
        _lib.call('mlc_conv_wgrad', _lib.ptr(dy), _lib.ptr(x), _lib.ptr(dw), N, H, W, C, Co, KH, KW,
                  stride, pack_pad(pad), dil, Ho, Wo, 0, int(accumulate), _lib.ptr(ws),
                  ws.numel() if ws is not None else 0, _lib.ptr(sc), _lib.ptr(sh), _lib.stream())
        return dw
    if in_affine is not None:
        x = bn_relu_input(x, in_affine)
    dwf = torch.nn.grad.conv2d_weight(x.permute(0, 3, 1, 2).float(), (Co, Ci, KH, KW),
                                      dy.permute(0, 3, 1, 2).float(), stride, pad, dil)
    dwf = dwf.permute(0, 2, 3, 1)
    if out is not None:
        if accumulate:
            out.add_(dwf.reshape(out.shape))
        else:
            out.copy_(dwf.reshape(out.shape))
        return out
    return dwf.contiguous()


NSTAT = _lib.DET_COPIES if _lib.DETERMINISTIC else 32


def stat_buffers(C, device):
    b = torch.zeros(2, NSTAT * C, device=device, dtype=torch.float32)
    return b[0], b[1]


BN_FUSED = os.environ.get('MLC_BN_FUSED', '1') == '1'


def _bn_fused_ok(C, ncopy):
    return BN_FUSED and not _lib.DETERMINISTIC and C % 8 == 0 and C >= 8 and 1 <= ncopy <= 64


def bn_fwd_apply(y, res, s1, s2, gamma, beta, save_mean, save_invstd, run_mean, run_var,
                 eps=1e-5, momentum=0.1, relu=True, out=None, scale=None, shift=None,
                 res_affine=None, apply=True):
    rows = y.numel() // y.shape[-1]
    C = y.shape[-1]
    ncopy = s1.numel() // C
    if _cuda(y):
        if scale is None:
            scale = torch.empty(2, C, device=y.device, dtype=torch.float32)
            scale, shift = scale[0], scale[1]
        if apply and _bn_fused_ok(C, ncopy):
            z = out if out is not None else torch.empty_like(y)
            rs, rh = res_affine if res_affine is not None else (None, None)
            _lib.call('mlc_bn_fwd_fused', _lib.ptr(y), _lib.ptr(res), _lib.ptr(z), _lib.ptr(s1), _lib.ptr(s2), ncopy,
                      _lib.ptr(gamma), _lib.ptr(beta), _lib.ptr(save_mean), _lib.ptr(save_invstd), _lib.ptr(scale),
                      _lib.ptr(shift), _lib.ptr(run_mean), _lib.ptr(run_var), _lib.ptr(rs), _lib.ptr(rh), rows, C,
                      float(eps), float(momentum), int(relu), _lib.stream())
            return z
        _lib.call('mlc_bn_finalize', _lib.ptr(s1), _lib.ptr(s2), ncopy, _lib.ptr(gamma), _lib.ptr(beta),
                  _lib.ptr(save_mean), _lib.ptr(save_invstd), _lib.ptr(scale), _lib.ptr(shift),
                  _lib.ptr(run_mean), _lib.ptr(run_var), rows, C, float(eps), float(momentum),
                  _lib.stream())
        if not apply:
            return None
        z = out if out is not None else torch.empty_like(y)
        rs, rh = res_affine if res_affine is not None else (None, None)
        _lib.call('mlc_bn_fwd_apply2', _lib.ptr(y), _lib.ptr(res), _lib.ptr(z), _lib.ptr(scale),
                  _lib.ptr(shift), _lib.ptr(rs), _lib.ptr(rh), rows, C, int(relu), _lib.stream())
        return z
    s1t = s1.reshape(ncopy, C).sum(0)
    s2t = s2.reshape(ncopy, C).sum(0)
    mean = s1t / rows
    var = (s2t / rows - mean * mean).clamp_min(0)
    inv = torch.rsqrt(var + eps)
    save_mean.copy_(mean)
    save_invstd.copy_(inv)
    if run_mean is not None:
        unb = var * rows / max(rows - 1, 1)
        run_mean.mul_(1 - momentum).add_(momentum * mean)
        run_var.mul_(1 - momentum).add_(momentum * unb)
    if scale is not None:
        scale.copy_(inv * gamma)
        shift.copy_(beta - mean * inv * gamma)
    if not apply:
        return None
    zf = (y.float() - mean) * (inv * gamma) + beta
    if res is not None:
        rf = res.float()
        if res_affine is not None:
            rf = rf * res_affine[0] + res_affine[1]
        zf = zf + rf
    if relu:
        zf = zf.clamp_min(0)
    z = zf.to(torch.bfloat16)
    if out is not None:
        out.copy_(z)
        return out
    return z


def bn_apply(y, res, scale, shift, relu=True, res_affine=None):
    rows = y.numel() // y.shape[-1]
    C = y.shape[-1]
    if _cuda(y):
        z = torch.empty_like(y)
        rs, rh = res_affine if res_affine is not None else (None, None)
        _lib.call('mlc_bn_fwd_apply2', _lib.ptr(y), _lib.ptr(res), _lib.ptr(z), _lib.ptr(scale),
                  _lib.ptr(shift), _lib.ptr(rs), _lib.ptr(rh), rows, C, int(relu), _lib.stream())
        return z
    zf = y.float() * scale + shift
    if res is not None:
        rf = res.float()
        if res_affine is not None:
            rf = rf * res_affine[0] + res_affine[1]
        zf = zf + rf
    if relu:
        zf = zf.clamp_min(0)
    return zf.to(torch.bfloat16)


def bn_bwd(dz, z, y, mean, invstd, gamma, want_dres=False, dgamma=None, dbeta=None, sums=None,
           zero_sums=True, coef=None, prereduced=False):
    rows = y.numel() // y.shape[-1]
    C = y.shape[-1]
    if prereduced:
        assert sums is not None
        z = None
    if _cuda(dz):
        if sums is None:
            sums = torch.zeros(NSTAT * 2 * C, device=dz.device, dtype=torch.float32)
        elif zero_sums and not prereduced:
            sums.zero_()
        if coef is None:
            coef = torch.empty(3 * C, device=dz.device, dtype=torch.float32)
        if not prereduced:
            _lib.call('mlc_bn_bwd_reduce', _lib.ptr(dz), _lib.ptr(z), _lib.ptr(y), _lib.ptr(mean),
                      _lib.ptr(sums), rows, C, _lib.stream())
        ncopy = NSTAT
        if _bn_fused_ok(C, ncopy):
            dy = torch.empty_like(y)
            dres = None
            if want_dres:
                dres = dz if prereduced else torch.empty_like(y)
            _lib.call('mlc_bn_bwd_fused', _lib.ptr(dz), _lib.ptr(z), _lib.ptr(y), _lib.ptr(mean), _lib.ptr(sums),
                      ncopy, _lib.ptr(invstd), _lib.ptr(gamma), _lib.ptr(dgamma), _lib.ptr(dbeta), _lib.ptr(dy),
                      _lib.ptr(None if prereduced else dres), rows, C, _lib.stream())
            return dy, dres
        _lib.call('mlc_bn_bwd_finalize', _lib.ptr(sums), _lib.ptr(invstd), _lib.ptr(gamma), _lib.ptr(coef),
                  _lib.ptr(dgamma), _lib.ptr(dbeta), rows, C, _lib.stream())
        dy = torch.empty_like(y)
        dres = None
        if want_dres:
            dres = dz if prereduced else torch.empty_like(y)
        _lib.call('mlc_bn_bwd_apply', _lib.ptr(dz), _lib.ptr(z), _lib.ptr(y), _lib.ptr(mean),
                  _lib.ptr(coef), _lib.ptr(dy), _lib.ptr(None if prereduced else dres), rows, C,
                  _lib.stream())
        return dy, dres
    d = dz.float().reshape(rows, C)
    if z is not None:
        d = d * (z.reshape(rows, C).float() > 0)
    yc = y.float().reshape(rows, C) - mean
    if prereduced:
        sv = sums.view(NSTAT, 2, C).sum(0)
        S1, S2 = sv[0], sv[1]
    else:
        S1 = d.sum(0)
        S2 = (d * yc).sum(0)
    if dgamma is not None:
        dgamma.copy_(S2 * invstd)
        dbeta.copy_(S1)
    k1 = gamma * invstd
    dyf = k1 * d - k1 * S1 / rows - k1 * invstd * invstd * S2 / rows * yc
    dy = dyf.reshape(y.shape).to(torch.bfloat16)
    dres = None
    if want_dres:
        dres = dz if prereduced else d.reshape(y.shape).to(torch.bfloat16)
    return dy, dres


FUSE_1X1_BWD = os.environ.get('MLC_FUSE_1X1_BWD', '1') == '1'


def conv1x1_bn_bwd_available(Cin, Cout) -> bool:
    return not _lib.DETERMINISTIC and bool(_lib.load().mlc_conv1x1_bn_bwd_ok(Cin, Cout))


def conv1x1_bn_bwd(dz, y, x, w, mean, invstd, gamma, sums, dgamma, dbeta, dw,
                   addend: Optional[torch.Tensor] = None, out: Optional[torch.Tensor] = None,
                   bn: Optional[BnBwdSpec] = None) -> torch.Tensor:
    Co, KH, KW, Ci = w.shape
    assert (KH, KW) == (1, 1) and y.shape[-1] == Co and x.shape[-1] == Ci, (w.shape, y.shape, x.shape)
    assert bn is None or (bn.mask is None and len(bn.ys) == 1 and bn.affine is not None)
    if _cuda(dz):
        rows = y.numel() // Co
        dx = out if out is not None else torch.empty_like(x)
        p = [None] * 5
        if bn is not None:
            (yk, mk, sk), (ak, hk) = bn.ys[0], bn.affine[0]
            p = [yk, mk, sk, ak, hk]
        _lib.call('mlc_conv1x1_bn_bwd', _lib.ptr(dz), _lib.ptr(y), _lib.ptr(x), _lib.ptr(w), _lib.ptr(mean),
                  _lib.ptr(invstd), _lib.ptr(gamma), _lib.ptr(sums), _lib.ptr(dgamma), _lib.ptr(dbeta),
                  _lib.ptr(dw), _lib.ptr(dx), _lib.ptr(addend), *[_lib.ptr(t) for t in p], rows, Ci, Co,
                  _lib.stream())
        return dx
    dy, _ = bn_bwd(dz, None, y, mean, invstd, gamma, dgamma=dgamma, dbeta=dbeta, sums=sums, prereduced=True)
    conv2d_wgrad(dy, x, w.shape, out=dw, accumulate=True)
    return conv2d_dgrad(dy, w, x.shape, addend=addend, out=out, bn=bn)


def pool_out_hw(H, W, k, s, p, ceil_mode=False):
    if not ceil_mode:
        return conv_out_hw(H, W, k, k, s, p, 1)

    def one(L):
        o = -(-(L + 2 * p - k) // s) + 1
        if (o - 1) * s >= L + p:
            o -= 1
        return o
    return one(H), one(W)


def maxpool_fwd(x, k=3, s=2, p=1, ceil_mode=False):
    N, H, W, C = x.shape
    Ho, Wo = pool_out_hw(H, W, k, s, p, ceil_mode)
    if _cuda(x):
        y = torch.empty(N, Ho, Wo, C, device=x.device, dtype=torch.bfloat16)
        idx = torch.empty(N, Ho, Wo, C, device=x.device, dtype=torch.uint8)
        _lib.call('mlc_maxpool_fwd', _lib.ptr(x), _lib.ptr(y), _lib.ptr(idx), N, H, W, C, Ho, Wo, k, s, p,
                  _lib.stream())
        return y, idx
    xf = x.permute(0, 3, 1, 2).float()
    yf, ind = F.max_pool2d(xf, k, s, p, ceil_mode=ceil_mode, return_indices=True)
    return yf.permute(0, 2, 3, 1).to(torch.bfloat16).contiguous(), ind


def maxpool_bwd(dy, idx, x_shape, k=3, s=2, p=1):
    N, H, W, C = x_shape
    _, Ho, Wo, _ = dy.shape
    if _cuda(dy):
        dx = torch.empty(N, H, W, C, device=dy.device, dtype=torch.bfloat16)
        _lib.call('mlc_maxpool_bwd', _lib.ptr(dy), _lib.ptr(idx), _lib.ptr(dx), N, H, W, C, Ho, Wo, k, s,
                  p, _lib.stream())
        return dx
    dyf = dy.permute(0, 3, 1, 2).float().reshape(N, C, -1)
    dxf = torch.zeros(N, C, H * W).scatter_add_(2, idx.reshape(N, C, -1), dyf)
    return dxf.reshape(N, C, H, W).permute(0, 2, 3, 1).to(torch.bfloat16).contiguous()

# ... 866 lines not shown
```

mlcomp_amd/ops/layers.py:

```python
from __future__ import annotations

import math
import os
from typing import List, Optional

import torch
import torch.nn as nn

from . import functional as Fn
from .arena import ParamArena, Slot

DGRAD_FIRST_ENV = os.environ.get('MLC_DGRAD_FIRST')
COMPACT_SHORTCUT_GRAD = os.environ.get('MLC_COMPACT_SHORTCUT_GRAD', '1') == '1'


class Workspace:

    def __init__(self):
        self._req: List[tuple] = []
        self.buf = None
        self.views = {}

    def request(self, key, n):
        self._req.append((key, int(n)))
        return key

    def finalize(self, device):
        total = sum((n + 63) // 64 * 64 for _, n in self._req) or 64
        self.buf = torch.zeros(total, device=device, dtype=torch.float32)
        off = 0
        for key, n in self._req:
            self.views[key] = self.buf[off:off + n]
            off += (n + 63) // 64 * 64

    def __getitem__(self, key):
        return self.views[key]

    def zero(self):
        self.buf.zero_()


class NativeContext:

    def __init__(self):
        self.arena = ParamArena()
        self.ws = Workspace()
        self.anchor = None
        self.training = True
        self.device = None
        self.grad_prezeroed = False
        self.wgrad_stream = None
        self.wt = Fn.WtTable() if os.environ.get('MLC_DGRAD_WT', '1') == '1' else None
        self.wt_stale = False
        self.wgrad_lag = int(os.environ.get('MLC_WGRAD_LAG', '0') or 0)
        self.wgrad_defer = False
        self._pending_wgrad = []
        self.dgrad_first = DGRAD_FIRST_ENV == '1'
        self.wgrad_slab = os.environ.get('MLC_WGRAD_SLAB', '1') != '0'
        self.deploy = False

    def default_wgrad_slab(self, on: bool):
        if os.environ.get('MLC_WGRAD_SLAB') is None:
            self.wgrad_slab = on

    def default_dgrad_first(self, on: bool):
        if DGRAD_FIRST_ENV is None:
            self.dgrad_first = on

    def finalize(self, device):
        self.device = torch.device(device)
        self.arena.finalize(device)
        self.ws.finalize(device)
        if self.wt is not None:
            self.wt.finalize(self.device)
        self.anchor = torch.zeros(1, device=device, requires_grad=True)
        self.arena.flush = self.flush_wgrad
        if self.device.type == 'cuda' and os.environ.get('MLC_WGRAD_STREAM', '1') in ('1', '2'):
            self.wgrad_stream = torch.cuda.Stream(self.device)
        self.default_wgrad_defer(False)

    def default_wgrad_defer(self, on: bool):
        env = os.environ.get('MLC_WGRAD_DEFER')
        self.wgrad_defer = (env == '1') if env is not None else on
        self.arena.grad_streams = [self.wgrad_stream] if (self.wgrad_defer and self.wgrad_stream) else []

    def flush_wgrad(self):
        if self.wgrad_defer and self.wgrad_stream is not None:
            cur = torch.cuda.current_stream(self.device)
            if cur != self.wgrad_stream:
                cur.wait_stream(self.wgrad_stream)
        self.join_wgrads(0)

    def default_wgrad_lag(self, n: int):
        if os.environ.get('MLC_WGRAD_LAG') is None:
            self.wgrad_lag = n

    def lag_wgrad(self, ev, keep, slots):
        self._pending_wgrad.append((ev, keep, slots))
        self.join_wgrads(self.wgrad_lag)

    def join_wgrads(self, keep_last: int):
        q = self._pending_wgrad
        while len(q) > keep_last:
            ev, _keep, slots = q.pop(0)
            cur = torch.cuda.current_stream(self.device)
            if cur != self.wgrad_stream:
                cur.wait_event(ev)
            for s in (slots if isinstance(slots, (list, tuple)) else (slots,)):
                self.arena.mark_ready(s)

    def refresh_wt(self):
        if self.wt is not None and self.training:
            self.wt.refresh()
        self.wt_stale = False


def flatten_bn_buffers(units) -> Optional[torch.Tensor]:
    units = [u for u in units if getattr(u, 'run_mean', None) is not None]
    if not units:
        return None
    flat = torch.empty(sum(2 * u.run_mean.numel() for u in units), device=units[0].run_mean.device)
    off = 0
    for u in units:
        C = u.run_mean.numel()
        flat[off:off + C].copy_(u.run_mean)
        flat[off + C:off + 2 * C].copy_(u.run_var)
        u.run_mean, u.run_var = flat[off:off + C], flat[off + C:off + 2 * C]
        off += 2 * C
    return flat


class ConvBN:

    def __init__(self, ctx: NativeContext, name: str, conv: nn.Conv2d, bn: nn.BatchNorm2d,
                 act: bool, cin_pad: Optional[int] = None, s2d: bool = False):
        assert conv.groups == 1, 'native ConvBN supports groups=1'
        self.ctx = ctx
        self.name = name
        Co, Ci, KH, KW = conv.weight.shape
        self.cin = Ci
        self.cin_p = cin_pad or Ci
        self.Co = Co
        self.k = (KH, KW)
        self.stride = conv.stride[0]
        self.pad = conv.padding[0]
        self.dil = conv.dilation[0]
        self.s2d = s2d
        if s2d:
            assert (KH, KW, self.stride, self.pad, self.dil) == (7, 7, 2, 3, 1) and Ci <= 3, \
                's2d stem needs a 7x7/2 pad-3 conv over <= 3 channels'
            self.k, self.stride, self.pad, self.cin_p = (4, 4), 1, 0, 16
            KH = KW = 4
        self.act = act
        self.eps = bn.eps
        self.momentum = bn.momentum if bn.momentum is not None else 0.1
        self.w = ctx.arena.weight(f'{name}.conv.weight', (Co, KH, KW, self.cin_p))
        self.wt_idx = None
        if ctx.wt is not None and not s2d:
            self.wt_idx = ctx.wt.add(self.w)
        self.gamma = ctx.arena.vector(f'{name}.bn.weight', (Co,))
        self.beta = ctx.arena.vector(f'{name}.bn.bias', (Co,))
        self._src = (conv, bn)
        self.k_s1 = ctx.ws.request(f'{name}.s1', Fn.NSTAT * Co)
        self.k_s2 = ctx.ws.request(f'{name}.s2', Fn.NSTAT * Co)
        self.k_bw = ctx.ws.request(f'{name}.bwd', Fn.NSTAT * 2 * Co)

    def load_from_torch(self):
        conv, bn = self._src
        dev = self.ctx.device
        if self.s2d:
            w = Fn.stem_w_to_s2d(conv.weight.detach().cpu())
            self._gmask = (Fn.stem_w_to_s2d(torch.ones(self.Co, self.cin, 7, 7)) != 0).float().to(dev)
        else:
            w = conv.weight.detach().permute(0, 2, 3, 1).float()
            if self.cin_p != self.cin:
                w = torch.nn.functional.pad(w, (0, self.cin_p - self.cin))
        self.w.master.copy_(w.to(dev))
        self.gamma.master.copy_(bn.weight.detach().to(dev))
        self.beta.master.copy_(bn.bias.detach().to(dev))
        self.run_mean = bn.running_mean.detach().clone().float().to(dev)
        self.run_var = bn.running_var.detach().clone().float().to(dev)
        Co = self.Co
        b = torch.zeros(7, Co, device=dev)
        self.save_mean, self.save_invstd, self.scale, self.shift = b[0], b[1], b[2], b[3]
        self.coef = b[4:7].reshape(-1)

    def export_to_torch(self):
        conv, bn = self._src
        if self.s2d:
            w = Fn.stem_w_from_s2d(self.w.master.detach().float().cpu(), self.cin)
        else:
            w = self.w.master[..., :self.cin].permute(0, 3, 1, 2).contiguous()
        conv.weight.data.copy_(w.to(conv.weight.device))
        bn.weight.data.copy_(self.gamma.master.to(bn.weight.device))
        bn.bias.data.copy_(self.beta.master.to(bn.bias.device))
        bn.running_mean.copy_(self.run_mean.to(bn.running_mean.device))
        bn.running_var.copy_(self.run_var.to(bn.running_var.device))

    def __call__(self, x, res=None):
        return _ConvBNFn.apply(x, res, self.ctx.anchor, self)

    def fwd(self, x, res=None, defer=False, in_affine=None):
        ws = self.ctx.ws
        if self.s2d and x.shape[-1] != 16:
            x = Fn.stem_s2d(x, 3)
        raff = None
        if isinstance(res, tuple):
            res, rs, rh = res
            raff = (rs, rh)
        if not self.ctx.training and self.ctx.deploy and self.folds():
            assert raff is None and in_affine is None and not defer, \
                f'{self.name}: deploy mode takes a materialised residual and input'
            if self._fold is None:
                self.refold()
            w_fold, b_fold = self._fold
            if self._conv1x1_res_ok(x):
                z = Fn.conv1x1_fwd_res(x, w_fold, b_fold, res, 3 if self.act else 0)
            else:
                z = Fn.conv2d_fwd_res(x, w_fold, b_fold, res, 3 if self.act else 0, self.stride, self.pad, self.dil)
            return z, (x, None, z)
        if not self.ctx.training:
            y = self._conv(x, None, in_affine)
            torch.rsqrt(self.run_var + self.eps, out=self.scale).mul_(self.gamma.master)
            torch.sub(self.beta.master, self.run_mean * self.scale, out=self.shift)
            if defer:
                return None, (x, y, None)
            z = Fn.bn_apply(y, res, self.scale, self.shift, self.act, res_affine=raff)
            return z, (x, y, z)
        s1, s2 = ws[self.k_s1], ws[self.k_s2]
        self.ctx.wt_stale = True
        y = self._conv(x, (s1, s2), in_affine)
        training = self.ctx.training
        z = Fn.bn_fwd_apply(y, res, s1, s2, self.gamma.master, self.beta.master, self.save_mean,
                            self.save_invstd, self.run_mean if training else None,
                            self.run_var if training else None, self.eps, self.momentum, self.act,
                            scale=self.scale, shift=self.shift, res_affine=raff, apply=not defer)
        return z, (x, y, z)

    _fold = None

    def folds(self) -> bool:
        return type(self) is ConvBN and not self.s2d

    def refold(self):
        if not self.folds():
            return
        with torch.no_grad():
            scale = self.gamma.master.float() * torch.rsqrt(self.run_var.float() + self.eps)
            w_fold = (self.w.master.float() * scale.view(-1, 1, 1, 1)).to(torch.bfloat16).contiguous()
            b_fold = (self.beta.master.float() - self.run_mean.float() * scale).contiguous()
            if self._fold is None:
                self._fold = (w_fold, b_fold)
            else:
                self._fold[0].copy_(w_fold)
                self._fold[1].copy_(b_fold)

    def _conv(self, x, stats, in_affine=None):
        if self.s2d and in_affine is None:
            return Fn.stem_conv_fwd(x, self.w.bf16, stats=stats)
        if stats is not None and in_affine is None and self._conv1x1_fwd_ok(x):
            return Fn.conv1x1_fwd(x, self.w.bf16, stats)
        return Fn.conv2d_fwd(x, self.w.bf16, self.stride, self.pad, self.dil, stats=stats, in_affine=in_affine)

    def _conv1x1_fwd_ok(self, x) -> bool:
        if not (Fn.CONV1X1_FWD and x.is_cuda and type(self) is ConvBN and not self.s2d):
            return False
        if self.k != (1, 1) or self.stride != 1 or self.pad != 0 or x.shape[-1] != self.cin_p:
            return False
        return Fn.conv1x1_fwd_available(self.cin_p, self.Co)

    def _conv1x1_res_ok(self, x) -> bool:
        if not (Fn.CONV1X1_RES and x.is_cuda and type(self) is ConvBN and not self.s2d):
            return False
        if self.k != (1, 1) or self.stride != 1 or self.pad != 0 or x.shape[-1] != self.cin_p:
            return False
        min_rows = Fn.conv1x1_res_min_rows(self.cin_p, self.Co)
        if min_rows is None or math.prod(x.shape[:-1]) < min_rows:
            return False
        return Fn.conv1x1_fwd_res_available(self.cin_p, self.Co)

    def _dgrad(self, dy, x_shape, addend=None, out=None, bn=None, saddend=None, compact=False):
        wt = None
        if self.wt_idx is not None:
            if self.ctx.wt_stale:
                raise RuntimeError('transposed filters are stale: the model must call '
                                   'ctx.refresh_wt() after its training forward pass')
            wt = self.ctx.wt[self.wt_idx]
        if compact:
            assert self.compact_dx() and addend is None and saddend is None and bn is None
            return Fn.conv2d_dgrad(dy, self.w.bf16, tuple(dy.shape[:3]) + (x_shape[3],), out=out, wt=wt)
        return Fn.conv2d_dgrad(dy, self.w.bf16, x_shape, self.stride, self.pad, self.dil,
                               addend=addend, out=out, bn=bn, wt=wt, strided_addend=saddend)

    def compact_dx(self) -> bool:
        return (COMPACT_SHORTCUT_GRAD and type(self) is ConvBN and not self.s2d and self.k == (1, 1)
                and self.pad == 0 and self.dil == 1 and self.stride > 1)

    def dgrad_covers_all(self) -> bool:
        return True

    def bn_target(self, rec):
        x, y, z = rec
        return (y, self.save_mean, self.ctx.ws[self.k_bw])

    def wgrad(self, dy, x, in_affine=None):
        Fn.conv2d_wgrad(dy, x, self.w.shape, self.stride, self.pad, self.dil, out=self.w.grad,
                        accumulate=self.ctx.grad_prezeroed, in_affine=in_affine, slab=self.ctx.wgrad_slab)
        if self.s2d:
            self.w.grad.mul_(self._gmask)

    def _fused_1x1_bwd_ok(self, dz, x, dgrad_bn) -> bool:
        if not (Fn.FUSE_1X1_BWD and dz.is_cuda and type(self) is ConvBN and not self.s2d):
            return False
        if self.k != (1, 1) or self.stride != 1 or self.pad != 0 or x.shape[-1] != self.cin_p:
            return False
        if dgrad_bn is not None and (dgrad_bn.mask is not None or len(dgrad_bn.ys) != 1
                                     or dgrad_bn.affine is None):
            return False
        return Fn.conv1x1_bn_bwd_available(self.cin_p, self.Co)

    def bwd(self, dz, rec, want_dres=False, dx_addend=None, need_dx=True, dx_out=None,
            prereduced=False, dgrad_bn=None, in_affine=None, defer: Optional[list] = None,
            dx_saddend=None, compact_dx=False):
        x, y, z = rec
        arena = self.ctx.arena
        if need_dx and prereduced and in_affine is None and dx_saddend is None \
                and self._fused_1x1_bwd_ok(dz, x, dgrad_bn):
            if not self.ctx.grad_prezeroed:
                self.w.grad.zero_()
            dx = Fn.conv1x1_bn_bwd(dz, y, x, self.w.bf16, self.save_mean, self.save_invstd,
                                   self.gamma.master, self.ctx.ws[self.k_bw], self.gamma.grad,
                                   self.beta.grad, self.w.grad, addend=dx_addend, out=dx_out, bn=dgrad_bn)
            arena.mark_ready(self.gamma)
            arena.mark_ready(self.beta)
            arena.mark_ready(self.w)
            return dx, (dz if want_dres else None)
        dy, dres = Fn.bn_bwd(dz, z if self.act else None, y, self.save_mean, self.save_invstd,
                             self.gamma.master, want_dres=want_dres, dgamma=self.gamma.grad,
                             dbeta=self.beta.grad, sums=self.ctx.ws[self.k_bw], zero_sums=False,
                             coef=self.coef, prereduced=prereduced)
        arena.mark_ready(self.gamma)
        arena.mark_ready(self.beta)
        side = self.ctx.wgrad_stream if need_dx else None
        if side is not None and torch.cuda.current_stream(self.ctx.device) == side:
            side = None
        fork = None
        if side is not None:
            main = torch.cuda.current_stream(self.ctx.device)
            fork = torch.cuda.Event()
            fork.record(main)
            if not self.ctx.dgrad_first:
                side.wait_event(fork)
                with Fn.side_stream(side):
                    self.wgrad(dy, x, in_affine)
        else:
            self.wgrad(dy, x, in_affine)
        dx = None
        if need_dx:
            dx = self._dgrad(dy, x.shape, addend=dx_addend, out=dx_out, bn=dgrad_bn, saddend=dx_saddend,
                             compact=compact_dx)
        if side is not None and self.ctx.dgrad_first:
            side.wait_event(fork)
            with Fn.side_stream(side):
                self.wgrad(dy, x, in_affine)
        if side is not None and defer is not None:
            defer.append((dy, x, self.w))
            return dx, dres
        if side is not None and self.ctx.wgrad_defer:
            dy.record_stream(side)
            x.record_stream(side)
            arena.mark_ready(self.w)
            return dx, dres
        if side is not None and self.ctx.wgrad_lag:
            ev = torch.cuda.Event()
            ev.record(side)
            self.ctx.lag_wgrad(ev, (dy, x), self.w)
            return dx, dres
        if side is not None:
            main.wait_stream(side)
        arena.mark_ready(self.w)
        return dx, dres


class ConvTBN(ConvBN):

    def __init__(self, ctx: NativeContext, name: str, conv: nn.ConvTranspose2d, bn: nn.BatchNorm2d, act: bool):
        assert conv.groups == 1 and conv.dilation[0] == conv.dilation[1], 'native ConvTBN: groups=1'
        assert conv.stride[0] == conv.stride[1] and conv.padding[0] == conv.padding[1]
        self.ctx = ctx
        self.name = name
        Cin, Cout, KH, KW = conv.weight.shape
        assert bn.num_features == Cout
        self.cin = self.cin_p = Cout
        self.Co = Cout
        self.k = (KH, KW)
        self.stride, self.pad, self.dil = conv.stride[0], conv.padding[0], conv.dilation[0]
        self.out_pad = conv.output_padding
        self.s2d = False
        self.act = act
        self.eps = bn.eps
        self.momentum = bn.momentum if bn.momentum is not None else 0.1
        self.w = ctx.arena.weight(f'{name}.conv.weight', (Cin, KH, KW, Cout))
        self.wt_idx = None
        self.gamma = ctx.arena.vector(f'{name}.bn.weight', (Cout,))
        self.beta = ctx.arena.vector(f'{name}.bn.bias', (Cout,))
        self._src = (conv, bn)
        self.k_s1 = ctx.ws.request(f'{name}.s1', Fn.NSTAT * Cout)
        self.k_s2 = ctx.ws.request(f'{name}.s2', Fn.NSTAT * Cout)
        self.k_bw = ctx.ws.request(f'{name}.bwd', Fn.NSTAT * 2 * Cout)

    def _bias(self):
        conv = self._src[0]
        return conv.bias.detach().float().to(self.ctx.device) if conv.bias is not None else None

    def load_from_torch(self):
        super().load_from_torch()
        b = self._bias()
        if b is not None:
            self.run_mean.sub_(b)

    def export_to_torch(self):
        super().export_to_torch()
        b = self._bias()
        if b is not None:
            bn = self._src[1]
            bn.running_mean.add_(b.to(bn.running_mean.device))

    def out_hw(self, H, W):
        KH, KW = self.k
        return ((H - 1) * self.stride - 2 * self.pad + self.dil * (KH - 1) + self.out_pad[0] + 1,
                (W - 1) * self.stride - 2 * self.pad + self.dil * (KW - 1) + self.out_pad[1] + 1)

    def _conv(self, x, stats, in_affine=None):
        assert in_affine is None
        return Fn.conv_transpose2d_fwd(x, self.w.bf16, self.out_hw(x.shape[1], x.shape[2]), self.stride,
                                       self.pad, self.dil, stats=stats)

    def _dgrad(self, dy, x_shape, addend=None, out=None, bn=None, saddend=None, compact=False):
        assert addend is None and out is None and bn is None and saddend is None and not compact, \
            'ConvTBN input gradient: plain conv'
        dx = Fn.conv2d_fwd(dy, self.w.bf16, self.stride, self.pad, self.dil)
        assert tuple(dx.shape) == tuple(x_shape), (dx.shape, x_shape)
        return dx

    def wgrad(self, dy, x, in_affine=None):
        assert in_affine is None
        Fn.conv2d_wgrad(x, dy, self.w.shape, self.stride, self.pad, self.dil, out=self.w.grad,
                        accumulate=self.ctx.grad_prezeroed)


class _ConvBNFn(torch.autograd.Function):
    @staticmethod
    def forward(ctx, x, res, anchor, m: ConvBN):
        z, rec = m.fwd(x, res)
        ctx.m = m
        ctx.has_res = res is not None
        ctx.save_for_backward(*rec)
        return z

    @staticmethod
    def backward(ctx, dz):
        m: ConvBN = ctx.m
        dx, dres = m.bwd(dz.contiguous(), ctx.saved_tensors, want_dres=ctx.has_res,
                         need_dx=ctx.needs_input_grad[0])
        return dx, dres, None, None


class ResidualBlock:

    def __init__(self, units: List[ConvBN], down: Optional[ConvBN]):
        self.units = units
        self.down = down
        self.ctx = units[0].ctx
        self.prev: Optional['ResidualBlock'] = None
        self.fuse_bn_bwd = True
        self.down_stream = os.environ.get('MLC_DOWN_STREAM', '1') == '1'
        mode = int(os.environ.get('MLC_FUSE_BN_FWD', '0'))
        one = lambda u: u.k == (1, 1) and u.stride == 1 and u.pad == 0
        self.fuse_into = [False] + [
            mode >= 1 and prev.act and (mode == 2 or (one(u) and (mode != 3 or u.cin <= 64)))
            for prev, u in zip(units[:-1], units[1:])]
        self.dout_prereduced = False
        self._last = None

    @property
    def fuse_bn_fwd(self) -> bool:
        return any(self.fuse_into)

    @fuse_bn_fwd.setter
    def fuse_bn_fwd(self, on: bool):
        self.fuse_into = [False] + [bool(on) and p.act for p in self.units[:-1]]

    def in_affines(self):
        return [None] + [(p.scale, p.shift) if f else None for p, f in zip(self.units[:-1], self.fuse_into[1:])]

    def __call__(self, x):
        if self.ctx.deploy and not self.ctx.training:
            return self.deploy_fwd(x)
        return _ResidualBlockFn.apply(x, self.ctx.anchor, self)

    def deploy_fwd(self, x):
        identity = x if self.down is None else self.down.fwd(x)[0]
        y = x
        for u in self.units[:-1]:
            y = u.fwd(y)[0]
        return self.units[-1].fwd(y, identity)[0]

    def output_bn_spec(self):
        rec, rd = self._last
        last = self.units[-1]
        ys = [last.bn_target(rec)]
        if self.down is not None and not self.down.act:
            ys.append(self.down.bn_target(rd))
            return Fn.BnBwdSpec(None, ys, affine=[(last.scale, last.shift),
                                                  (self.down.scale, self.down.shift)])
        if self.down is not None:
            ys.append(self.down.bn_target(rd))
        return Fn.BnBwdSpec(rec[2], ys)


class _ResidualBlockFn(torch.autograd.Function):
    @staticmethod
    def forward(ctx, x, anchor, blk: ResidualBlock):
        recs = []
        side = blk.ctx.wgrad_stream if (blk.down is not None and blk.down_stream) else None
        if side is not None:
            main = torch.cuda.current_stream(blk.ctx.device)
            side.wait_stream(main)
        if blk.down is not None:
            if side is not None:
                with Fn.side_stream(side):
                    _, rd = blk.down.fwd(x, defer=not blk.down.act)
            else:
                _, rd = blk.down.fwd(x, defer=not blk.down.act)
            identity = rd[2] if blk.down.act else (rd[1], blk.down.scale, blk.down.shift)
        else:
            identity, rd = x, None
        y = x
        affs = blk.in_affines()
        for i, u in enumerate(blk.units[:-1]):
            if blk.fuse_into[i + 1]:
                _, r = u.fwd(y, defer=True, in_affine=affs[i])
                y = r[1]
            else:
                y, r = u.fwd(y, in_affine=affs[i])
            recs.append(r)
        if side is not None:
            main.wait_stream(side)
        out, r = blk.units[-1].fwd(y, identity, in_affine=affs[-1])
        recs.append(r)
        blk._last = (r, rd)
        ctx.blk = blk
        ctx.n = len(recs)
        flat = [t for r in recs for t in r]
        if rd is not None:
            flat += list(rd)
        ctx.save_for_backward(*flat)
        return out

    @staticmethod
    def backward(ctx, dout):
        blk: ResidualBlock = ctx.blk
        saved = ctx.saved_tensors
        recs = [saved[3 * i:3 * i + 3] for i in range(ctx.n)]
        rd = saved[3 * ctx.n:3 * ctx.n + 3] if blk.down is not None else None
        dout = dout.contiguous()
        need_dx = ctx.needs_input_grad[0]
        pre = blk.dout_prereduced
        blk.dout_prereduced = False
        units = blk.units
        fuse = blk.fuse_bn_bwd
        affs = blk.in_affines()
        if blk.fuse_bn_fwd:
            assert fuse, 'the BN-apply fusion needs the fused BN-backward reductions (z is not stored)'

        def spec_for(i):
            u = units[i]
            if not fuse or not units[i + 1].dgrad_covers_all():
                return None
            if u.act:
                return Fn.BnBwdSpec(None, [u.bn_target(recs[i])], affine=[(u.scale, u.shift)])
            return Fn.BnBwdSpec(None, [u.bn_target(recs[i])])

        side = units[0].ctx.wgrad_stream
        pend = [] if side is not None and os.environ.get('MLC_WGRAD_STREAM') == '2' else None
        sp = spec_for(len(units) - 2) if len(units) > 1 else None
        d, dres = units[-1].bwd(dout, recs[-1], want_dres=True, prereduced=pre, dgrad_bn=sp,
                                in_affine=affs[-1], defer=pend)
        fused = sp is not None
        down_side = side if (blk.down is not None and pend is None and blk.down_stream) else None
        short = dres
        compact = need_dx and blk.down is not None and blk.down.compact_dx()
        if down_side is not None:
            main = torch.cuda.current_stream(units[0].ctx.device)
            short_shape = tuple(dres.shape[:3]) + (rd[0].shape[3],) if compact else rd[0].shape
            short_buf = torch.empty(short_shape, device=rd[0].device, dtype=rd[0].dtype) if need_dx else None
            down_side.wait_stream(main)
            with Fn.side_stream(down_side):
                short, _ = blk.down.bwd(dres, rd, need_dx=need_dx, prereduced=pre, dx_out=short_buf,
                                        compact_dx=compact)
        for i in range(len(units) - 2, 0, -1):
            sp = spec_for(i - 1)
            d, _ = units[i].bwd(d, recs[i], prereduced=fused, dgrad_bn=sp, in_affine=affs[i], defer=pend)
            fused = sp is not None
        if down_side is not None:
            main.wait_stream(down_side)
        elif blk.down is not None:
            short, _ = blk.down.bwd(dres, rd, need_dx=need_dx, prereduced=pre, defer=pend, compact_dx=compact)
        prev_spec = None
        if need_dx and fuse and blk.prev is not None and blk.prev._last is not None \
                and units[0].dgrad_covers_all():
            prev_spec = blk.prev.output_bn_spec()
        if compact:
            dx, _ = units[0].bwd(d, recs[0], dx_saddend=(short, blk.down.stride), need_dx=need_dx,
                                 prereduced=fused, dgrad_bn=prev_spec, defer=pend)
        else:
            dx, _ = units[0].bwd(d, recs[0], dx_addend=short if need_dx else None, need_dx=need_dx,
                                 dx_out=short if (need_dx and blk.down is not None) else None,
                                 prereduced=fused, dgrad_bn=prev_spec, defer=pend)
        if prev_spec is not None:
            blk.prev.dout_prereduced = True
        if pend:
            torch.cuda.current_stream(units[0].ctx.device).wait_stream(side)
            for _, _, w in pend:
                units[0].ctx.arena.mark_ready(w)
            pend.clear()
        return dx, None, None


class MaxPool:
    def __init__(self, k=3, s=2, p=1):
        self.k, self.s, self.p = k, s, p

    def __call__(self, x, anchor):
        return _MaxPoolFn.apply(x, anchor, self)


class _MaxPoolFn(torch.autograd.Function):
    @staticmethod
    def forward(ctx, x, anchor, m):
        y, idx = Fn.maxpool_fwd(x, m.k, m.s, m.p)
        ctx.m = m
        ctx.xshape = tuple(x.shape)
        ctx.save_for_backward(idx)
        return y

    @staticmethod
    def backward(ctx, dy):
        (idx,) = ctx.saved_tensors
        m = ctx.m
        return Fn.maxpool_bwd(dy.contiguous(), idx, ctx.xshape, m.k, m.s, m.p), None, None


class StemPool:

    def __init__(self, stem: ConvBN):
        assert stem.act, 'StemPool fuses the stem ReLU'
        self.stem = stem
        self.ctx = stem.ctx

    def __call__(self, x):
        return _StemPoolFn.apply(x, self.ctx.anchor, self)


class _StemPoolFn(torch.autograd.Function):
    @staticmethod
    def forward(ctx, x, anchor, m: StemPool):
        st = m.stem
        if not st.ctx.training:
            z, _ = st.fwd(x)
            out, _ = Fn.maxpool_fwd(z)
            return out
        _, (x_, y, _) = st.fwd(x, defer=True)
        out, idx = Fn.stem_pool_fwd(y, st.scale, st.shift)
        ctx.m = m
        ctx.save_for_backward(x_, y, idx)
        return out

    @staticmethod
    def backward(ctx, dp):
        st: ConvBN = ctx.m.stem
        x, y, idx = ctx.saved_tensors
        arena = st.ctx.arena
        dy = Fn.stem_pool_bwd(dp.contiguous(), idx, y, st.save_mean, st.save_invstd, st.gamma.master,
                              st.gamma.grad, st.beta.grad, st.ctx.ws[st.k_bw], st.coef)
        arena.mark_ready(st.gamma)
        arena.mark_ready(st.beta)
        st.wgrad(dy, x)
        arena.mark_ready(st.w)
        return None, None, None


class ClassifierHead:

    def __init__(self, ctx: NativeContext, name: str, fc: nn.Linear, smoothing: float = 0.0):
        self.ctx = ctx
        self.name = name
        self.fc = fc
        self.O, self.I = fc.weight.shape
        self.Op = (self.O + 7) // 8 * 8
        self.w = ctx.arena.weight(f'{name}.weight', (self.Op, self.I))
        self.b = ctx.arena.vector(f'{name}.bias', (self.Op,))
        self.smoothing = smoothing
        self.k_loss = ctx.ws.request(f'{name}.loss', 1)
# ... 52 lines not shown
```

Before: 14640 images/s.

## Store packed ReLU sign bits in BN forward for cheaper dgrad masking

For identity-shortcut residual blocks that feed a later block, the last BN-apply kernel now also writes a 1-bit-per-element ReLU positivity mask. The following block's dgrad epilogue reads those bits in place of the full bf16 output tensor when masking the gradient. This cuts the backward epilogue from reading 16 bytes per 8 channels to 1 byte. The cost is an extra byte write per 8 elements in forward and an extra allocation per block. It also disables the affine-recompute path and the fused 1x1 BN-bwd path for those blocks.

```diff
diff --git a/csrc/kernels/batchnorm.hip b/csrc/kernels/batchnorm.hip
--- a/csrc/kernels/batchnorm.hip
+++ b/csrc/kernels/batchnorm.hip
@@ -42,7 +42,7 @@
 bn_fwd_apply_kernel(const bf16* __restrict__ y, const bf16* __restrict__ res, bf16* __restrict__ z,
                     const float* __restrict__ scale_, const float* __restrict__ shift_,
                     const float* __restrict__ rscale_, const float* __restrict__ rshift_,
-                    long rows, int C, int relu) {
+                    long rows, int C, int relu, unsigned char* __restrict__ zbits) {
   const int G = C >> 3;
   const long gtid = (long)blockIdx.x * NT + threadIdx.x;
   const long stride = (long)gridDim.x * NT;
@@ -81,7 +81,11 @@
 #pragma unroll
         for (int j = 0; j < 8; ++j) f[j] = fmaxf(f[j], 0.f);
       }
-      if (i < total) *reinterpret_cast<uint4*>(z + i * 8) = pack8(f);
+      if (i < total) {
+        const uint4 zv = pack8(f);
+        *reinterpret_cast<uint4*>(z + i * 8) = zv;
+        if (zbits) zbits[i] = (unsigned char)posbits8(zv);
+      }
     }
   }
 }
@@ -263,7 +267,8 @@
                     float* __restrict__ scale_out, float* __restrict__ shift_out,
                     float* __restrict__ run_mean, float* __restrict__ run_var,
                     const float* __restrict__ rscale_, const float* __restrict__ rshift_,
-                    long rows, int C, float eps, float momentum, int relu) {
+                    long rows, int C, float eps, float momentum, int relu,
+                    unsigned char* __restrict__ zbits) {
   __shared__ float lsc[FG * 8], lsh[FG * 8], red[2][NT];
   const int G = C >> 3;
   int gb, nslices;
@@ -332,7 +337,9 @@
 #pragma unroll
         for (int j = 0; j < 8; ++j) f[j] = fmaxf(f[j], 0.f);
       }
-      *reinterpret_cast<uint4*>(z + (r * G + cg) * 8) = pack8(f);
+      const uint4 zv = pack8(f);
+      *reinterpret_cast<uint4*>(z + (r * G + cg) * 8) = zv;
+      if (zbits) zbits[r * G + cg] = (unsigned char)posbits8(zv);
     }
   }
 }
@@ -477,21 +484,27 @@
   return hipGetLastError();
 }
 
-MLC_EXPORT int mlc_bn_fwd_apply2(const bf16* y, const bf16* res, bf16* z, const float* scale,
-                                 const float* shift, const float* rscale, const float* rshift, long rows,
-                                 int C, int relu, hipStream_t st) {
+MLC_EXPORT int mlc_bn_fwd_apply2_bits(const bf16* y, const bf16* res, bf16* z, const float* scale,
+                                      const float* shift, const float* rscale, const float* rshift, long rows,
+                                      int C, int relu, unsigned char* zbits, hipStream_t st) {
   if (!shape_ok(C) || (rscale && !rshift)) return -1;
   const dim3 grid(grid_for(rows, C));
   if (g_unroll >= 4)
     hipLaunchKernelGGL(bn_fwd_apply_kernel<4>, grid, dim3(NT), 0, st, y, res, z, scale, shift, rscale, rshift,
-                       rows, C, relu);
+                       rows, C, relu, zbits);
   else if (g_unroll == 2)
     hipLaunchKernelGGL(bn_fwd_apply_kernel<2>, grid, dim3(NT), 0, st, y, res, z, scale, shift, rscale, rshift,
-                       rows, C, relu);
+                       rows, C, relu, zbits);
   else
     hipLaunchKernelGGL(bn_fwd_apply_kernel<1>, grid, dim3(NT), 0, st, y, res, z, scale, shift, rscale, rshift,
-                       rows, C, relu);
-  return hipGetLastError();
+                       rows, C, relu, zbits);
+  return hipGetLastError();
+}
+
+MLC_EXPORT int mlc_bn_fwd_apply2(const bf16* y, const bf16* res, bf16* z, const float* scale,
+                                 const float* shift, const float* rscale, const float* rshift, long rows,
+                                 int C, int relu, hipStream_t st) {
+  return mlc_bn_fwd_apply2_bits(y, res, z, scale, shift, rscale, rshift, rows, C, relu, nullptr, st);
 }
 
 MLC_EXPORT int mlc_bn_fwd_apply(const bf16* y, const bf16* res, bf16* z, const float* scale,
@@ -525,18 +538,27 @@
   return hipGetLastError();
 }
 
+MLC_EXPORT int mlc_bn_fwd_fused_bits(const bf16* y, const bf16* res, bf16* z, const float* sum, const float* sumsq,
+                                     int ncopy, const float* gamma, const float* beta, float* save_mean,
+                                     float* save_invstd, float* scale, float* shift, float* run_mean,
+                                     float* run_var, const float* rscale, const float* rshift, long rows, int C,
+                                     float eps, float momentum, int relu, unsigned char* zbits, hipStream_t st) {
+  if (!fused_ok(C, ncopy) || (rscale && !rshift) || rows < 1) return -1;
+#define MLC_BNF(U) hipLaunchKernelGGL(bn_fwd_fused_kernel<U>, dim3(fused_grid(rows, C)), dim3(NT), 0, st, y, res, z, \
+                                      sum, sumsq, ncopy, gamma, beta, save_mean, save_invstd, scale, shift, run_mean, \
+                                      run_var, rscale, rshift, rows, C, eps, momentum, relu, zbits)
+  if (g_unroll >= 4) MLC_BNF(4); else if (g_unroll == 2) MLC_BNF(2); else MLC_BNF(1);
+#undef MLC_BNF
+  return hipGetLastError();
+}
+
 MLC_EXPORT int mlc_bn_fwd_fused(const bf16* y, const bf16* res, bf16* z, const float* sum, const float* sumsq,
                                 int ncopy, const float* gamma, const float* beta, float* save_mean,
                                 float* save_invstd, float* scale, float* shift, float* run_mean, float* run_var,
                                 const float* rscale, const float* rshift, long rows, int C, float eps,
                                 float momentum, int relu, hipStream_t st) {
-  if (!fused_ok(C, ncopy) || (rscale && !rshift) || rows < 1) return -1;
-#define MLC_BNF(U) hipLaunchKernelGGL(bn_fwd_fused_kernel<U>, dim3(fused_grid(rows, C)), dim3(NT), 0, st, y, res, z, \
-                                      sum, sumsq, ncopy, gamma, beta, save_mean, save_invstd, scale, shift, run_mean, \
-                                      run_var, rscale, rshift, rows, C, eps, momentum, relu)
-  if (g_unroll >= 4) MLC_BNF(4); else if (g_unroll == 2) MLC_BNF(2); else MLC_BNF(1);
-#undef MLC_BNF
-  return hipGetLastError();
+  return mlc_bn_fwd_fused_bits(y, res, z, sum, sumsq, ncopy, gamma, beta, save_mean, save_invstd, scale, shift,
+                               run_mean, run_var, rscale, rshift, rows, C, eps, momentum, relu, nullptr, st);
 }
 
 MLC_EXPORT int mlc_bn_bwd_fused(const bf16* dz, const bf16* z, const bf16* y, const float* mean, const float* sums,
diff --git a/csrc/kernels/common.h b/csrc/kernels/common.h
--- a/csrc/kernels/common.h
+++ b/csrc/kernels/common.h
@@ -53,6 +53,15 @@
   return r;
 }
 
+static __device__ __forceinline__ unsigned posbits8(const uint4& u) {
+  float f[8];
+  unpack8(u, f);
+  unsigned b = 0;
+#pragma unroll
+  for (int e = 0; e < 8; ++e) b |= (f[e] > 0.f ? 1u : 0u) << e;
+  return b;
+}
+
 static __device__ __forceinline__ uint4 ldg16(const void* p) {
   typedef unsigned u32x4 __attribute__((ext_vector_type(4)));
   const u32x4 v = *reinterpret_cast<const u32x4*>(p);
diff --git a/csrc/kernels/igemm.hip b/csrc/kernels/igemm.hip
--- a/csrc/kernels/igemm.hip
+++ b/csrc/kernels/igemm.hip
@@ -542,6 +542,7 @@
   const float* msc0 = nullptr; const float* msh0 = nullptr;
   const float* msc1 = nullptr; const float* msh1 = nullptr;
   int ncopy = NSTAT;
+  const unsigned char* mbits = nullptr;
 };
 
 __device__ __forceinline__ float erf_from_exp(float x, float e) {
@@ -652,7 +653,7 @@
     const int nc = n0 + c * 8;
     const bool red = !kDense && bn.y0 != nullptr;
     float mu0[8], mu1[8], s1[8], s2[8], t2[8], ma0[8], mb0[8], ma1[8], mb1[8];
-    const bool aff = red && !bn.mask && bn.msc0, aff1 = aff && bn.msc1;
+    const bool aff = red && !bn.mask && !bn.mbits && bn.msc0, aff1 = aff && bn.msc1;
     if (red) {
       const int ncl = nc < N ? nc : 0;
 #pragma unroll
@@ -685,6 +686,7 @@
     constexpr int UMAX = kDense ? 4 : 8;
     constexpr int U = ITERS < UMAX ? ITERS : UMAX;
     const bool has_add = addend != nullptr, has_mask = red && bn.mask, has_y1 = red && bn.y1;
+    const bool has_bits = red && !bn.mask && bn.mbits;
     constexpr bool kSAdd = HasStridedAdd<RowMap>::value;
 #pragma unroll 1
     for (int it0 = 0; it0 < ITERS; it0 += U) {
@@ -713,7 +715,9 @@
           aa[u] = has_add ? ldg16(addend + off[u]) : zero;
         }
         if constexpr (!kDense) {
-          zz[u] = has_mask ? ldg16(bn.mask + off[u]) : zero;
+          zz[u] = has_mask   ? ldg16(bn.mask + off[u])
+                  : has_bits ? make_uint4((unsigned)bn.mbits[off[u] >> 3], 0u, 0u, 0u)
+                             : zero;
           p0[u] = red ? ldg16(bn.y0 + off[u]) : zero;
           p1[u] = has_y1 ? ldg16(bn.y1 + off[u]) : zero;
         }
@@ -746,6 +750,10 @@
               unpack8(zz[u], z);
 #pragma unroll
               for (int e = 0; e < 8; ++e) a[e] = z[e] > 0.f ? a[e] : 0.f;
+            } else if (has_bits) {
+              const unsigned zb = zz[u].x;
+#pragma unroll
+              for (int e = 0; e < 8; ++e) a[e] = (zb >> e) & 1u ? a[e] : 0.f;
             } else if (aff) {
               float y[8], q[8];
               unpack8(p0[u], y);
@@ -1688,6 +1696,7 @@
   if (add.S < 1 || (add.compact && add.same)) return -1;
   if (bn.y0 && g_mlc_det && ((long)N * H * W + 63) / 64 > g_mlc_ncopy) return -2;
   if (bn.msc0 && (!bn.msh0 || !bn.y0 || (bn.msc1 && (!bn.msh1 || !bn.y1)))) return -1;
+  if (bn.mbits && (bn.mask || bn.msc0 || !bn.y0)) return -1;
   if (bn.y0 && (!bn.mean0 || !bn.sums0 || (bn.y1 && (!bn.mean1 || !bn.sums1)))) return -1;
   return 0;
 }
@@ -1737,9 +1746,9 @@
                            const float* bn_mean0, float* bn_sums0, const bf16* bn_y1,
                            const float* bn_mean1, float* bn_sums1, const float* bn_msc0,
                            const float* bn_msh0, const float* bn_msc1, const float* bn_msh1,
-                           float* sum, float* sumsq, hipStream_t st) {
+                           const unsigned char* bn_mbits, float* sum, float* sumsq, hipStream_t st) {
   const BnBwdEpi bn{bn_mask, bn_y0, bn_mean0, bn_sums0, bn_y1, bn_mean1, bn_sums1,
-                    bn_msc0, bn_msh0, bn_msc1, bn_msh1, g_mlc_ncopy};
+                    bn_msc0, bn_msh0, bn_msc1, bn_msh1, g_mlc_ncopy, bn_mbits};
   if (const int rc = dgrad_check(bn, add, N, H, W, C, Co, KH, KW, stride, sum, sumsq)) return rc;
   const ConvGeom g = mkgeom(N, H, W, C, Co, KH, KW, stride, pad, dil, Ho, Wo);
   if (KH == 1 && KW == 1 && stride == 1 && pad == 0) {
@@ -1752,6 +1761,18 @@
   return dgrad_classes<MkConvDgradB>(dy, w, dx, add, bn, g, pad, sum, sumsq, st);
 }
 
+MLC_EXPORT int mlc_conv_dgrad_bits(const bf16* dy, const bf16* w, bf16* dx, const bf16* addend, const bf16* sadd,
+                                   int sadd_stride, int N, int H, int W, int C, int Co, int KH, int KW,
+                                   int stride, int pad, int dil, int Ho, int Wo, const bf16* bn_mask,
+                                   const bf16* bn_y0, const float* bn_mean0, float* bn_sums0, const bf16* bn_y1,
+                                   const float* bn_mean1, float* bn_sums1, const float* bn_msc0,
+                                   const float* bn_msh0, const float* bn_msc1, const float* bn_msh1,
+                                   const unsigned char* bn_mbits, hipStream_t st) {
+  return conv_dgrad_impl(dy, w, dx, DgradAddend{addend, sadd, sadd_stride}, N, H, W, C, Co, KH, KW, stride, pad, dil,
+                         Ho, Wo, bn_mask, bn_y0, bn_mean0, bn_sums0, bn_y1, bn_mean1, bn_sums1, bn_msc0, bn_msh0,
+                         bn_msc1, bn_msh1, bn_mbits, nullptr, nullptr, st);
+}
+
 MLC_EXPORT int mlc_conv_dgrad(const bf16* dy, const bf16* w, bf16* dx, const bf16* addend, int N,
                               int H, int W, int C, int Co, int KH, int KW, int stride, int pad,
                               int dil, int Ho, int Wo, const bf16* bn_mask, const bf16* bn_y0,
@@ -1759,9 +1780,9 @@
                               const float* bn_mean1, float* bn_sums1, const float* bn_msc0,
                               const float* bn_msh0, const float* bn_msc1, const float* bn_msh1,
                               hipStream_t st) {
-  return conv_dgrad_impl(dy, w, dx, DgradAddend{addend}, N, H, W, C, Co, KH, KW, stride, pad, dil, Ho, Wo, bn_mask,
-                         bn_y0, bn_mean0, bn_sums0, bn_y1, bn_mean1, bn_sums1, bn_msc0, bn_msh0, bn_msc1, bn_msh1,
-                         nullptr, nullptr, st);
+  return mlc_conv_dgrad_bits(dy, w, dx, addend, nullptr, 1, N, H, W, C, Co, KH, KW, stride, pad, dil, Ho, Wo, bn_mask,
+                             bn_y0, bn_mean0, bn_sums0, bn_y1, bn_mean1, bn_sums1, bn_msc0, bn_msh0, bn_msc1,
+                             bn_msh1, nullptr, st);
 }
 
 MLC_EXPORT int mlc_conv_dgrad_sadd(const bf16* dy, const bf16* w, bf16* dx, const bf16* addend, const bf16* sadd,
@@ -1771,9 +1792,9 @@
                                    const float* bn_mean1, float* bn_sums1, const float* bn_msc0,
                                    const float* bn_msh0, const float* bn_msc1, const float* bn_msh1,
                                    hipStream_t st) {
-  return conv_dgrad_impl(dy, w, dx, DgradAddend{addend, sadd, sadd_stride}, N, H, W, C, Co, KH, KW, stride, pad, dil,
-                         Ho, Wo, bn_mask, bn_y0, bn_mean0, bn_sums0, bn_y1, bn_mean1, bn_sums1, bn_msc0, bn_msh0,
-                         bn_msc1, bn_msh1, nullptr, nullptr, st);
+  return mlc_conv_dgrad_bits(dy, w, dx, addend, sadd, sadd_stride, N, H, W, C, Co, KH, KW, stride, pad, dil, Ho, Wo,
+                             bn_mask, bn_y0, bn_mean0, bn_sums0, bn_y1, bn_mean1, bn_sums1, bn_msc0, bn_msh0,
+                             bn_msc1, bn_msh1, nullptr, st);
 }
 
 MLC_EXPORT int mlc_conv_tr_fwd(const bf16* x, const bf16* w, bf16* y, float* sum, float* sumsq, int N, int Hi,
@@ -1785,7 +1806,7 @@
     return -1;
   return conv_dgrad_impl(x, w, y, DgradAddend{}, N, Ho, Wo, Cout, Cin, KH, KW, stride, pad, dil, Hi, Wi, nullptr,
                          nullptr, nullptr, nullptr, nullptr, nullptr, nullptr, nullptr, nullptr, nullptr,
-                         nullptr, sum, sumsq, st);
+                         nullptr, nullptr, sum, sumsq, st);
 }
 
 static int conv_dgrad_t_impl(const bf16* dy, const bf16* wt, bf16* dx, const DgradAddend& add, int N,
@@ -1794,9 +1815,9 @@
                              const float* bn_mean0, float* bn_sums0, const bf16* bn_y1,
                              const float* bn_mean1, float* bn_sums1, const float* bn_msc0,
                              const float* bn_msh0, const float* bn_msc1, const float* bn_msh1,
-                             hipStream_t st) {
+                             const unsigned char* bn_mbits, hipStream_t st) {
   const BnBwdEpi bn{bn_mask, bn_y0, bn_mean0, bn_sums0, bn_y1, bn_mean1, bn_sums1,
-                    bn_msc0, bn_msh0, bn_msc1, bn_msh1, g_mlc_ncopy};
+                    bn_msc0, bn_msh0, bn_msc1, bn_msh1, g_mlc_ncopy, bn_mbits};
   if (const int rc = dgrad_check(bn, add, N, H, W, C, Co, KH, KW, stride, nullptr, nullptr)) return rc;
   int pad_h, pad_w;
   unpack_pad(pad, pad_h, pad_w);
@@ -1816,6 +1837,18 @@
   return dgrad_classes<MkConvDgradBT>(dy, wt, dx, add, bn, g, pad, nullptr, nullptr, st);
 }
 
+MLC_EXPORT int mlc_conv_dgrad_t_bits(const bf16* dy, const bf16* wt, bf16* dx, const bf16* addend, const bf16* sadd,
+                                     int sadd_stride, int N, int H, int W, int C, int Co, int KH, int KW,
+                                     int stride, int pad, int dil, int Ho, int Wo, const bf16* bn_mask,
+                                     const bf16* bn_y0, const float* bn_mean0, float* bn_sums0, const bf16* bn_y1,
+                                     const float* bn_mean1, float* bn_sums1, const float* bn_msc0,
+                                     const float* bn_msh0, const float* bn_msc1, const float* bn_msh1,
+                                     const unsigned char* bn_mbits, hipStream_t st) {
+  return conv_dgrad_t_impl(dy, wt, dx, DgradAddend{addend, sadd, sadd_stride}, N, H, W, C, Co, KH, KW, stride, pad,
+                           dil, Ho, Wo, bn_mask, bn_y0, bn_mean0, bn_sums0, bn_y1, bn_mean1, bn_sums1, bn_msc0,
+                           bn_msh0, bn_msc1, bn_msh1, bn_mbits, st);
+}
+
 MLC_EXPORT int mlc_conv_dgrad_t(const bf16* dy, const bf16* wt, bf16* dx, const bf16* addend, int N,
                                 int H, int W, int C, int Co, int KH, int KW, int stride, int pad,
                                 int dil, int Ho, int Wo, const bf16* bn_mask, const bf16* bn_y0,
@@ -1823,9 +1856,9 @@
                                 const float* bn_mean1, float* bn_sums1, const float* bn_msc0,
                                 const float* bn_msh0, const float* bn_msc1, const float* bn_msh1,
                                 hipStream_t st) {
-  return conv_dgrad_t_impl(dy, wt, dx, DgradAddend{addend}, N, H, W, C, Co, KH, KW, stride, pad, dil, Ho, Wo,
-                           bn_mask, bn_y0, bn_mean0, bn_sums0, bn_y1, bn_mean1, bn_sums1, bn_msc0, bn_msh0, bn_msc1,
-                           bn_msh1, st);
+  return mlc_conv_dgrad_t_bits(dy, wt, dx, addend, nullptr, 1, N, H, W, C, Co, KH, KW, stride, pad, dil, Ho, Wo,
+                               bn_mask, bn_y0, bn_mean0, bn_sums0, bn_y1, bn_mean1, bn_sums1, bn_msc0, bn_msh0,
+                               bn_msc1, bn_msh1, nullptr, st);
 }
 
 MLC_EXPORT int mlc_conv_dgrad_t_sadd(const bf16* dy, const bf16* wt, bf16* dx, const bf16* addend, const bf16* sadd,
@@ -1835,9 +1868,9 @@
                                      const float* bn_mean1, float* bn_sums1, const float* bn_msc0,
                                      const float* bn_msh0, const float* bn_msc1, const float* bn_msh1,
                                      hipStream_t st) {
-  return conv_dgrad_t_impl(dy, wt, dx, DgradAddend{addend, sadd, sadd_stride}, N, H, W, C, Co, KH, KW, stride, pad,
-                           dil, Ho, Wo, bn_mask, bn_y0, bn_mean0, bn_sums0, bn_y1, bn_mean1, bn_sums1, bn_msc0,
-                           bn_msh0, bn_msc1, bn_msh1, st);
+  return mlc_conv_dgrad_t_bits(dy, wt, dx, addend, sadd, sadd_stride, N, H, W, C, Co, KH, KW, stride, pad, dil, Ho,
+                               Wo, bn_mask, bn_y0, bn_mean0, bn_sums0, bn_y1, bn_mean1, bn_sums1, bn_msc0, bn_msh0,
+                               bn_msc1, bn_msh1, nullptr, st);
 }
 
 namespace {
diff --git a/mlcomp_amd/ops/_lib.py b/mlcomp_amd/ops/_lib.py
--- a/mlcomp_amd/ops/_lib.py
+++ b/mlcomp_amd/ops/_lib.py
@@ -21,6 +21,8 @@
     'mlc_conv_dgrad_t': [vp] * 4 + [i32] * 12 + [vp] * 11 + [vp],
     'mlc_conv_dgrad_sadd': [vp] * 5 + [i32] * 13 + [vp] * 11 + [vp],
     'mlc_conv_dgrad_t_sadd': [vp] * 5 + [i32] * 13 + [vp] * 11 + [vp],
+    'mlc_conv_dgrad_bits': [vp] * 5 + [i32] * 13 + [vp] * 12 + [vp],
+    'mlc_conv_dgrad_t_bits': [vp] * 5 + [i32] * 13 + [vp] * 12 + [vp],
     'mlc_bilinear_up_fwd': [vp, vp] + [i32] * 6 + [vp],
     'mlc_bilinear_up_bwd': [vp, vp] + [i32] * 6 + [vp],
     'mlc_gn_relu_fwd': [vp, vp, vp, vp, vp] + [i32] * 4 + [f32, vp],
@@ -73,9 +75,11 @@
     'mlc_bn_finalize': [vp, vp, i32] + [vp] * 8 + [i64, i32, f32, f32, vp],
     'mlc_bn_fwd_apply': [vp] * 5 + [i64, i32, i32, vp],
     'mlc_bn_fwd_apply2': [vp] * 7 + [i64, i32, i32, vp],
+    'mlc_bn_fwd_apply2_bits': [vp] * 7 + [i64, i32, i32, vp, vp],
     'mlc_bn_bwd_reduce': [vp] * 5 + [i64, i32, vp],
     'mlc_bn_bwd_finalize': [vp] * 6 + [i64, i32, vp],
     'mlc_bn_fwd_fused': [vp] * 5 + [i32] + [vp] * 10 + [i64, i32, f32, f32, i32, vp],
+    'mlc_bn_fwd_fused_bits': [vp] * 5 + [i32] + [vp] * 10 + [i64, i32, f32, f32, i32, vp, vp],
     'mlc_bn_bwd_fused': [vp] * 5 + [i32] + [vp] * 6 + [i64, i32, vp],
     'mlc_bnact_fused': [vp] * 5 + [i32] + [vp] * 10 + [i64, i32, f32, f32, i32, f32, vp, i64, vp, i32, vp, i64, vp],
     'mlc_bn_bwd_apply': [vp] * 7 + [i64, i32, vp],
diff --git a/mlcomp_amd/ops/functional.py b/mlcomp_amd/ops/functional.py
--- a/mlcomp_amd/ops/functional.py
+++ b/mlcomp_amd/ops/functional.py
@@ -162,12 +162,25 @@
 
 class BnBwdSpec:
 
-    def __init__(self, mask, ys, affine=None):
+    def __init__(self, mask, ys, affine=None, bits=None):
         assert 1 <= len(ys) <= 2
         assert affine is None or (mask is None and len(affine) == len(ys))
+        assert bits is None or (mask is None and affine is None and bits.dtype == torch.uint8)
         self.mask = mask
         self.ys = list(ys)
         self.affine = list(affine) if affine is not None else None
+        self.bits = bits
+
+
+def pack_relu_bits(z: torch.Tensor) -> torch.Tensor:
+    m = (z.float() > 0).reshape(-1, 8).to(torch.uint8)
+    wgt = torch.tensor([1, 2, 4, 8, 16, 32, 64, 128], dtype=torch.uint8, device=z.device)
+    return (m * wgt).sum(1, dtype=torch.int32).to(torch.uint8)
+
+
+def unpack_relu_bits(bits: torch.Tensor, C: int) -> torch.Tensor:
+    sh = torch.arange(8, device=bits.device, dtype=torch.int32)
+    return ((bits.reshape(-1, 1).to(torch.int32) >> sh) & 1).reshape(-1, C).float()
 
 
 def wt_flip_transpose(w: torch.Tensor) -> torch.Tensor:
@@ -263,8 +276,14 @@
         add = [_lib.ptr(addend)]
         if strided_addend is not None:
             name, add = name + '_sadd', [None, _lib.ptr(sadd), S]
+        tail = []
+        if bn is not None and bn.bits is not None:
+            assert bn.bits.dtype == torch.uint8 and bn.bits.is_contiguous() and bn.bits.numel() == N * H * W * C // 8
+            if strided_addend is None:
+                add = add + [None, 1]
+            name, tail = name.replace('_sadd', '') + '_bits', [_lib.ptr(bn.bits)]
         _lib.call(name, _lib.ptr(dy), _lib.ptr(filt), _lib.ptr(dx), *add, N, H, W, C, Co, KH, KW, stride,
-                  pack_pad(pad), dil, Ho, Wo, *[_lib.ptr(t) for t in b], _lib.stream())
+                  pack_pad(pad), dil, Ho, Wo, *[_lib.ptr(t) for t in b], *tail, _lib.stream())
         return dx
     if wt is not None and isinstance(pad, int) and dgrad_as_fwd_conv(KH, KW, stride, pad, dil):
         dxf = F.conv2d(dy.permute(0, 3, 1, 2).float(), wt.permute(0, 3, 1, 2).float(), None, 1,
@@ -283,6 +302,8 @@
     if bn is not None:
         if bn.mask is not None:
             dxf = dxf * (bn.mask.float() > 0)
+        elif bn.bits is not None:
+            dxf = dxf * unpack_relu_bits(bn.bits, C).view(N, H, W, C)
         elif bn.affine is not None:
             q = sum(yk.float() * ak + hk for (yk, _, _), (ak, hk) in zip(bn.ys, bn.affine))
             dxf = dxf * (q > 0)
@@ -432,10 +453,13 @@
 
 def bn_fwd_apply(y, res, s1, s2, gamma, beta, save_mean, save_invstd, run_mean, run_var,
                  eps=1e-5, momentum=0.1, relu=True, out=None, scale=None, shift=None,
-                 res_affine=None, apply=True):
+                 res_affine=None, apply=True, zbits=None):
     rows = y.numel() // y.shape[-1]
     C = y.shape[-1]
     ncopy = s1.numel() // C
+    if zbits is not None:
+        assert apply and zbits.dtype == torch.uint8 and zbits.is_contiguous() and zbits.numel() == rows * C // 8
+    sfx, zb = ('_bits', [_lib.ptr(zbits)]) if zbits is not None else ('', [])
     if _cuda(y):
         if scale is None:
             scale = torch.empty(2, C, device=y.device, dtype=torch.float32)
@@ -443,10 +467,10 @@
         if apply and _bn_fused_ok(C, ncopy):
             z = out if out is not None else torch.empty_like(y)
             rs, rh = res_affine if res_affine is not None else (None, None)
-            _lib.call('mlc_bn_fwd_fused', _lib.ptr(y), _lib.ptr(res), _lib.ptr(z), _lib.ptr(s1), _lib.ptr(s2), ncopy,
+            _lib.call('mlc_bn_fwd_fused' + sfx, _lib.ptr(y), _lib.ptr(res), _lib.ptr(z), _lib.ptr(s1), _lib.ptr(s2), ncopy,
                       _lib.ptr(gamma), _lib.ptr(beta), _lib.ptr(save_mean), _lib.ptr(save_invstd), _lib.ptr(scale),
                       _lib.ptr(shift), _lib.ptr(run_mean), _lib.ptr(run_var), _lib.ptr(rs), _lib.ptr(rh), rows, C,
-                      float(eps), float(momentum), int(relu), _lib.stream())
+                      float(eps), float(momentum), int(relu), *zb, _lib.stream())
             return z
         _lib.call('mlc_bn_finalize', _lib.ptr(s1), _lib.ptr(s2), ncopy, _lib.ptr(gamma), _lib.ptr(beta),
                   _lib.ptr(save_mean), _lib.ptr(save_invstd), _lib.ptr(scale), _lib.ptr(shift),
@@ -456,8 +480,8 @@
             return None
         z = out if out is not None else torch.empty_like(y)
         rs, rh = res_affine if res_affine is not None else (None, None)
-        _lib.call('mlc_bn_fwd_apply2', _lib.ptr(y), _lib.ptr(res), _lib.ptr(z), _lib.ptr(scale),
-                  _lib.ptr(shift), _lib.ptr(rs), _lib.ptr(rh), rows, C, int(relu), _lib.stream())
+        _lib.call('mlc_bn_fwd_apply2' + sfx, _lib.ptr(y), _lib.ptr(res), _lib.ptr(z), _lib.ptr(scale),
+                  _lib.ptr(shift), _lib.ptr(rs), _lib.ptr(rh), rows, C, int(relu), *zb, _lib.stream())
         return z
     s1t = s1.reshape(ncopy, C).sum(0)
     s2t = s2.reshape(ncopy, C).sum(0)
@@ -484,6 +508,8 @@
     if relu:
         zf = zf.clamp_min(0)
     z = zf.to(torch.bfloat16)
+    if zbits is not None:
+        zbits.copy_(pack_relu_bits(z))
     if out is not None:
         out.copy_(z)
         return out
diff --git a/mlcomp_amd/ops/layers.py b/mlcomp_amd/ops/layers.py
--- a/mlcomp_amd/ops/layers.py
+++ b/mlcomp_amd/ops/layers.py
@@ -12,6 +12,7 @@
 
 DGRAD_FIRST_ENV = os.environ.get('MLC_DGRAD_FIRST')
 COMPACT_SHORTCUT_GRAD = os.environ.get('MLC_COMPACT_SHORTCUT_GRAD', '1') == '1'
+RELU_BITS = os.environ.get('MLC_RELU_BITS', '1') == '1'
 
 
 class Workspace:
@@ -200,7 +201,8 @@
     def __call__(self, x, res=None):
         return _ConvBNFn.apply(x, res, self.ctx.anchor, self)
 
-    def fwd(self, x, res=None, defer=False, in_affine=None):
+    def fwd(self, x, res=None, defer=False, in_affine=None, zbits=None):
+        assert zbits is None or (self.ctx.training and not defer)
         ws = self.ctx.ws
         if self.s2d and x.shape[-1] != 16:
             x = Fn.stem_s2d(x, 3)
@@ -234,7 +236,7 @@
         z = Fn.bn_fwd_apply(y, res, s1, s2, self.gamma.master, self.beta.master, self.save_mean,
                             self.save_invstd, self.run_mean if training else None,
                             self.run_var if training else None, self.eps, self.momentum, self.act,
-                            scale=self.scale, shift=self.shift, res_affine=raff, apply=not defer)
+                            scale=self.scale, shift=self.shift, res_affine=raff, apply=not defer, zbits=zbits)
         return z, (x, y, z)
 
     _fold = None
@@ -314,8 +316,8 @@
             return False
         if self.k != (1, 1) or self.stride != 1 or self.pad != 0 or x.shape[-1] != self.cin_p:
             return False
-        if dgrad_bn is not None and (dgrad_bn.mask is not None or len(dgrad_bn.ys) != 1
-                                     or dgrad_bn.affine is None):
+        if dgrad_bn is not None and (dgrad_bn.mask is not None or dgrad_bn.bits is not None
+                                     or len(dgrad_bn.ys) != 1 or dgrad_bn.affine is None):
             return False
         return Fn.conv1x1_bn_bwd_available(self.cin_p, self.Co)
 
@@ -472,8 +474,10 @@
         self.units = units
         self.down = down
         self.ctx = units[0].ctx
-        self.prev: Optional['ResidualBlock'] = None
+        self._prev: Optional['ResidualBlock'] = None
+        self._next = 0
         self.fuse_bn_bwd = True
+        self.relu_bits = RELU_BITS
         self.down_stream = os.environ.get('MLC_DOWN_STREAM', '1') == '1'
         mode = int(os.environ.get('MLC_FUSE_BN_FWD', '0'))
         one = lambda u: u.k == (1, 1) and u.stride == 1 and u.pad == 0
@@ -484,6 +488,21 @@
         self._last = None
 
     @property
+    def prev(self) -> Optional['ResidualBlock']:
+        return self._prev
+
+    @prev.setter
+    def prev(self, blk: Optional['ResidualBlock']):
+        if self._prev is not None:
+            self._prev._next -= 1
+        self._prev = blk
+        if blk is not None:
+            blk._next += 1
+
+    def wants_relu_bits(self) -> bool:
+        return self.relu_bits and self.down is None and self._next > 0 and self.ctx.training
+
+    @property
     def fuse_bn_fwd(self) -> bool:
         return any(self.fuse_into)
 
@@ -507,9 +526,11 @@
         return self.units[-1].fwd(y, identity)[0]
 
     def output_bn_spec(self):
-        rec, rd = self._last
+        rec, rd, bits = self._last
         last = self.units[-1]
         ys = [last.bn_target(rec)]
+        if bits is not None:
+            return Fn.BnBwdSpec(None, ys, bits=bits)
         if self.down is not None and not self.down.act:
             ys.append(self.down.bn_target(rd))
             return Fn.BnBwdSpec(None, ys, affine=[(last.scale, last.shift),
@@ -547,9 +568,12 @@
             recs.append(r)
         if side is not None:
             main.wait_stream(side)
-        out, r = blk.units[-1].fwd(y, identity, in_affine=affs[-1])
+        bits = None
+        if blk.wants_relu_bits():
+            bits = torch.empty(identity.numel() // 8, device=x.device, dtype=torch.uint8)
+        out, r = blk.units[-1].fwd(y, identity, in_affine=affs[-1], zbits=bits)
         recs.append(r)
-        blk._last = (r, rd)
+        blk._last = (r, rd, bits)
         ctx.blk = blk
         ctx.n = len(recs)
         flat = [t for r in recs for t in r]
```

Measured after the change: 14730 images/s (median of 6 runs). Within noise of the previous version (+0.6%).
